# Agricultural-Robotics-Bonn/pagnerf

Measured on AMD Instinct MI355X. Metric: rays/sec (train step) on BUP20-shape scene, higher is better.
Workload: dtype bf16

## Files before the change

include/pagnerf_hip.h:

```cpp
#ifndef PAGNERF_HIP_H
#define PAGNERF_HIP_H

#include <stdint.h>

#ifdef __cplusplus
extern "C" {
#endif

#define PAG_ABI_VERSION 14

enum { PAG_F32 = 0, PAG_F16 = 1, PAG_BF16 = 2 };
enum { PAG_OK = 0, PAG_ERR_ARG = -1, PAG_ERR_LAUNCH = -2, PAG_ERR_UNSUPPORTED = -3 };
enum { PAG_ACT_NONE = 0, PAG_ACT_SIGMOID = 1, PAG_ACT_SOFTMAX = 2 };
enum { PAG_MLP_MFMA_BF16 = 0, PAG_MLP_FP32 = 1 };
enum { PAG_BG_BLACK = 0, PAG_BG_WHITE = 1 };
enum { PAG_LAYOUT_STRIDED = 0, PAG_LAYOUT_XCD8 = 1 };
enum { PAG_ENC_HALF_COORDS = 1 };
#define PAG_MAX_LEVELS 32
#define PAG_MAX_FEATS 64

int pag_abi_version(void);
const char *pag_last_error_string(void);


// ... 44 lines not shown
                            float *d_xyz, void *workspace, int64_t workspace_bytes, int flags, void *stream);
int pag_permuto_encode_bwd_xyz(const float *xyz, int64_t M, const void *tables, int table_dtype,
                               const void *grad_out, int grad_dtype, int64_t g_stride_m,
                               int64_t g_stride_c, int layout, int n_levels, int n_feat,
                               uint32_t capacity, const float *scale_factor_host,
                               const float *shift_host, const float *feat_scale_host, float *d_xyz,
                               void *workspace, int64_t workspace_bytes, int flags, void *stream);

int64_t pag_encode_bwd_workspace_bytes(int64_t M, int n_levels, int n_feat, int n_vertices,
                                       int64_t rows_per_level);


struct pag_head_composite_args;
typedef struct pag_mlp_fwd_args {
    const void *x1; int x1_dtype; int k1;
    int x1_layout; int x1_levels; int x1_feats;
    const float *x2; int k2p; const int32_t *x2_index;
    int in_dim; int n_layers; int out_dim;
    const float *W[3]; const float *b[3];
    int out_act;
    void *out; int out_dtype;
    void *hidden_save[2];
    int mode;
    float *softmax_stats;
    float *x1_col0_relu;
    const struct pag_mlp_fwd_args *pair;
    const struct pag_head_composite_args *composite;
    const struct pag_mlp_fwd_args *x1_producer;
} pag_mlp_fwd_args;
typedef struct pag_head_composite_args {
    const int64_t *pack_start; const int32_t *ray_of_pack; int64_t P;
    const float *weights;
    const float *alpha;
    float *out;
    int64_t n_samples;
} pag_head_composite_args;
int pag_mlp_fwd(const pag_mlp_fwd_args *args, int64_t M, void *stream);
int pag_mlp_fwd_pair_supported(const pag_mlp_fwd_args *args, const pag_mlp_fwd_args *pair);
int pag_mlp_fwd_composite_supported(const pag_mlp_fwd_args *args, int64_t M);
int pag_mlp_fwd_producer_supported(const pag_mlp_fwd_args *args, const pag_mlp_fwd_args *producer, int64_t M);

typedef struct pag_mlp_bwd_args {
    const void *grad_out; const void *out; int out_dtype; int out_act;
    int k1; int in_dim; int n_layers; int out_dim;
    int x1_layout; int x1_levels; int x1_feats;
    const float *W[3];
    const void *hidden_save[2];
    void *dz[3];
    void *dx1; int dx1_dtype;
    int mode;
    const float *g_ray; const float *g_scale; const int32_t *g_index;
    const float *softmax_stats; const float *b_last;
    int dx1_accumulate;
    const float *dx1_col0_add;
    const float *dx1_col0_gate;
    const float *g_ray_scale;
    const void *x1; int x1_dtype; const float *x2; int k2p; const int32_t *x2_index;
    float *wgrad_workspace; int64_t wgrad_workspace_bytes;
    float *dW[3]; float *db[3];
    const float *b[3];
    const struct pag_mlp_bwd_args *pair;
    float *dz0_slots;
} pag_mlp_bwd_args;
int pag_mlp_bwd(const pag_mlp_bwd_args *args, int64_t M, void *stream);
int64_t pag_mlp_dz0_slots_bytes(int64_t M, int64_t R);
int pag_mlp_dz0_slots_sum(const int64_t *pack_start, int64_t R, const float *slots, float *out, void *stream);
int pag_mlp_bwd_fused_supported(const pag_mlp_bwd_args *args);
#define PAG_MLP_FUSED_WIDE_MAX_M ((int64_t)1 << 24)
int64_t pag_mlp_bwd_fused_workspace_bytes(const pag_mlp_bwd_args *args, int64_t M);
int pag_mlp_bwd_pair_supported(const pag_mlp_bwd_args *args, const pag_mlp_bwd_args *pair);

int pag_affine_xcd8_fwd(const void *x, int64_t M, int x_levels, int x_feats, const float *W, const float *b, int n_out, int in_dim,
                        float *out, void *stream);
int pag_affine_xcd8_bwd_dx(const float *grad_out, int64_t M, int x_levels, int x_feats, const float *W, int n_out, int in_dim, void *dx,
                           void *stream);

int pag_head_composite_fwd(const int64_t *pack_start, const int32_t *ray_of_pack, int64_t P,
                           const void *hidden, const float *W_last, const float *b_last, int out_dim,
                           const float *softmax_stats, const float *weights, const float *alpha,
                           float *out, int64_t n_samples, void *stream);

int pag_mlp_wgrad_blocks(int64_t M);
int pag_mlp_wgrad(const void *dz, int dz_cols, int n_out, const void *a1, int a1_dtype,
                  int a1_layout, int k1, const float *a2, int k2p, const int32_t *a2_index, int n_in,
                  float *slabs, int n_blocks, int64_t M, void *stream);

int pag_mlp_wgrad_finish(const float *slabs, int n_blocks, int n_out, int n_in, int a1_layout,
                         int a1_levels, int a1_feats, float *dW, float *db, void *stream);

typedef struct pag_wgrad_layer {
    const void *dz;
    int dz_cols, n_out;
    const void *a1;
    int a1_dtype, a1_layout, k1;
    const float *a2;
    int k2p;
    const int32_t *a2_index;
    int n_in;
    float *slabs;
    int n_blocks;
    int a1_levels, a1_feats;
    float *dW, *db;
} pag_wgrad_layer;
int pag_mlp_wgrad_batch(const pag_wgrad_layer *layers, int n_layers, int64_t M, void *stream);


int pag_raymarch_count(const float *origins, const float *dirs, int64_t N, int S,
                       const float *tvals, const float *jitter, float dist_min, float dist_max,
                       const uint32_t *occupancy_bits, int blas_level, int32_t *counts,
                       void *stream);
int pag_pack_offsets(const int32_t *counts, int64_t N, int64_t *pack_start, int64_t *total_host, void *stream);
int pag_pad_packed(const int64_t *pack_start, int64_t N, int64_t capacity, int samples_per_entry, float *samples, float *depths,
                   float *deltas, int32_t *ridx_sample, int32_t *ridx_entry, int64_t *ridx64, int32_t *pidx,
                   uint8_t *boundary, int64_t *pack_start_clamped, void *stream);

int pag_pack_offsets_pad(const int32_t *counts, int64_t N, int64_t *pack_start, int64_t *total_host, int64_t capacity,
                         int samples_per_entry, float *samples, float *depths, float *deltas, int32_t *ridx_sample,
                         int32_t *ridx_entry, int64_t *ridx64, int32_t *pidx, uint8_t *boundary, int64_t *pack_start_clamped,
                         const float *dirs_src, float *dirs_dst, void *stream);

int pag_copy_batch(int n, void *const *dst, const void *const *src, const int64_t *nbytes, void *stream);

int pag_view_embed(const float *dirs, int64_t R, int n_freq, int width, float *out, void *stream);

int pag_raymarch_pack(const float *origins, const float *dirs, int64_t N, int S,
                      const float *tvals, const float *jitter, float dist_min, float dist_max,
                      const uint32_t *occupancy_bits, int blas_level, const int64_t *offsets,
                      int32_t *ridx, int32_t *pidx, float *samples, float *depths, float *deltas,
                      uint8_t *boundary, int64_t *ridx64, void *stream);

int pag_raymarch_voxel_count(const float *origins, const float *dirs, int64_t N, int samples_per_voxel,
                             float dist_min, float dist_max, const uint32_t *occupancy_bits,
                             const uint32_t *occupancy_coarse, int blas_level, float max_travel,
                             int32_t *counts, void *stream);
int pag_raymarch_voxel_pack(const float *origins, const float *dirs, int64_t N, int samples_per_voxel,
                            float dist_min, float dist_max, const uint32_t *occupancy_bits,
                            const uint32_t *occupancy_coarse, int blas_level, float max_travel,
                            const int64_t *offsets, int32_t *ridx, int32_t *pidx, float *samples,
                            float *depths, float *deltas, uint8_t *boundary, int32_t *ridx_sample,
                            int64_t *ridx64, void *stream);

int64_t pag_raymarch_voxel_nugget_capacity(int blas_level);
int pag_raymarch_voxel_count_nuggets(const float *origins, const float *dirs, int64_t N, int samples_per_voxel,
                                     float dist_min, float dist_max, const uint32_t *occupancy_bits,
                                     const uint32_t *occupancy_coarse, int blas_level, float max_travel,
                                     int32_t *counts, float *nugget_t, int32_t *nugget_cell, void *stream);
int pag_raymarch_voxel_pack_nuggets(const float *origins, const float *dirs, int64_t N, int samples_per_voxel,
                                    const int64_t *offsets, const float *nugget_t, const int32_t *nugget_cell, int blas_level,
                                    int32_t *ridx, int32_t *pidx, float *samples, float *depths, float *deltas,
                                    uint8_t *boundary, int32_t *ridx_sample, int64_t *ridx64, void *stream);

int64_t pag_occupancy_coarse_bytes(int blas_level);
int pag_occupancy_coarse(const uint32_t *occupancy_bits, int blas_level, uint32_t *coarse, void *stream);

int pag_occupancy_update(const float *density, int64_t density_stride, float *occupancy,
                         uint32_t *occupancy_bits, int64_t num_cells, float decay,
                         float min_density, void *stream);


int pag_composite_fwd(const int64_t *pack_start, const int32_t *ray_of_pack, int64_t P,
                      const float *sigma, const float *deltas, const float *depths,
                      const float *rgb, int bg_color, float *weights, float *out_alpha,
                      float *out_rgb, float *out_depth, uint8_t *out_hit, int64_t n_samples, void *stream);

int pag_composite_bwd(const int64_t *pack_start, const int32_t *ray_of_pack, int64_t P,
                      const float *sigma, const float *deltas, const float *depths,
                      const float *rgb, int bg_color, const float *weights,
                      const float *out_alpha, const float *g_rgb, const float *g_depth,
                      const float *g_alpha, float *d_sigma, float *d_rgb, int64_t n_samples, void *stream);

int pag_ray_sample_grad(const int64_t *pack_start, const int32_t *ray_of_pack, int64_t P, const float *grad_samples, const float *depths,
                        float *out, void *stream);

int pag_composite_feats_fwd(const int64_t *pack_start, const int32_t *ray_of_pack, int64_t P,
                            const float *weights, const float *alpha, const void *feats,
                            int feat_dtype, int C, float *out, void *stream);
int pag_composite_feats_bwd(const int64_t *pack_start, const int32_t *ray_of_pack, int64_t P,
                            const float *weights, const float *alpha, const float *g_out, int C,
                            void *d_feats, int feat_dtype, void *stream);


int pag_label_sums(const void *values, int value_dtype, int64_t P, int64_t row_stride, int col0, int C,
                   const int64_t *labels_gt, const uint8_t *row_mask, const int64_t *label_list, int K,
                   float *sums, int32_t *counts, void *stream);

int pag_assign_cost(const float *prob, int B, int64_t P, int64_t image_stride, int64_t row_stride, int n_cols, int col0,
                    const int64_t *labels_gt, int max_rows, float *sums_ws, int32_t *counts_ws, int32_t *info, int64_t *labels,
                    float *cost, const float *points, float id_slope, float id_x_limit, int id_margin, float *psums_ws,
                    int32_t *pcounts_ws, int32_t *id_lo_hi, void *stream);
int pag_assign_solve(const float *cost, int B, int max_rows, int n_ids, const int32_t *info, const int32_t *id_lo_hi, int64_t *targets, int32_t *status,
                     void *stream);
int pag_assign_nll_fwd(const float *prob, int B, int64_t P, int64_t image_stride, int64_t row_stride, int n_cols,
                       const int64_t *labels_gt, const uint8_t *stuff_mask, const int64_t *labels, const int64_t *targets,
                       const int32_t *info, int max_rows, int64_t default_label, int64_t *virt, float *loss, uint8_t *valid,
                       int32_t *wrong, void *stream);
int pag_assign_nll_bwd(const float *prob, int B, int64_t P, int64_t image_stride, int64_t row_stride, int n_cols,
                       const int64_t *virt, const uint8_t *valid, const int32_t *wrong, const float *grad, float *d_prob,
                       void *stream);

int64_t pag_segment_reg_workspace_bytes(int B, int64_t P);
int pag_segment_reg_fwd(const float *prob, int B, int64_t P, int64_t image_stride, int64_t row_stride, int n_cols, float eps,
                        const int64_t *labels, void *workspace, int64_t workspace_bytes, float *out, void *stream);
int pag_segment_reg_bwd(const float *prob, int B, int64_t P, int64_t image_stride, int64_t row_stride, int n_cols, float eps,
                        const void *workspace, int64_t workspace_bytes, const float *grad, float *d_prob, void *stream);


int64_t pag_supcon_workspace_bytes(int B, int64_t P, int D);
int pag_supcon_fwd(const void *features, int dtype, int B, int64_t P, int D, int64_t image_stride, int64_t row_stride, const int64_t *labels,
                   const uint8_t *anchor_mask, float temperature, float base_temperature, float pos_weight, float neg_weight, void *workspace,
                   int64_t workspace_bytes, float *loss, void *stream);
int pag_supcon_bwd(int dtype, int B, int64_t P, int D, float temperature, float base_temperature, float pos_weight, float neg_weight, void *workspace,
                   int64_t workspace_bytes, const float *grad_loss, void *d_features, void *stream);


int64_t pag_meanshift_workspace_bytes(int B, int64_t P, int D);

int pag_meanshift_fit(const void *features, int dtype, int B, int64_t P, int D, int64_t image_stride, int64_t row_stride, const int64_t *labels,
                      double quantile, int max_iter, int stages, void *workspace, int64_t workspace_bytes, float *means, double *bandwidth,
                      float *centers, int32_t *info, void *stream);

int pag_meanshift_predict(const void *x, int dtype, int64_t N, int D, int64_t row_stride, const float *centers, int C, int64_t *labels_out,
                          void *stream);

enum { PAG_I32 = 3, PAG_I64 = 4 };

int64_t pag_panoptic_pq_workspace_bytes(int B, int64_t H, int64_t W, int n_cat);

int pag_panoptic_pq_update(const void *preds, int preds_dtype, const int64_t *preds_strides, const void *target, int target_dtype,
                           const int64_t *target_strides, int B, int64_t H, int64_t W, const int64_t *cat_ids, const int32_t *cat_cont, int n_cat,
                           int n_things, int allow_unknown, void *workspace, int64_t workspace_bytes, double *iou_sum, int32_t *true_positives,
                           int32_t *false_positives, int32_t *false_negatives, int32_t *state_flags, void *stream);

int64_t pag_panoptic_clean_workspace_bytes(int64_t H, int64_t W);

int pag_panoptic_clean(const void *ids, int dtype, int64_t H, int64_t W, int64_t stride_y, int64_t stride_x, int num_openings, int outlier_rejection,
                       int64_t min_area, double std_threshold, void *workspace, int64_t workspace_bytes, void *out, void *stream);

int pag_confusion_matrix(const void *preds, int preds_dtype, const int64_t *preds_strides, const void *target, int target_dtype,
                         const int64_t *target_strides, const int64_t *shape, int C, int64_t *confmat, void *stream);


int64_t pag_map_workspace_bytes(int64_t n);

int pag_map_points(const float *params, int64_t C, const int32_t *cam, int64_t n_cam, int64_t rays_per_camera, const float *origins_c,
                   const float *dirs_c, int64_t ray0, int64_t n, const float *depth, const float *alpha, const uint8_t *hit,
                   const float *density, const float *rgb, const float *inst, int I, int64_t inst_stride, const int64_t *ids_in,
                   float min_density, float min_alpha, float depth_min, float depth_max, float *points, float *color, int64_t *ids_out,
                   int64_t cap, int64_t *count, void *workspace, int64_t workspace_bytes, void *stream);

int pag_map_select(const float *points_in, int64_t n, const float *value, float threshold, const float *inst, int I, int64_t inst_stride,
                   const int64_t *ids_in, float *points, int64_t *ids_out, int64_t cap, int64_t *count, void *workspace,
                   int64_t workspace_bytes, void *stream);


int64_t pag_render_loss_workspace_bytes(void);
int pag_render_loss_fwd(const float *rgb, const float *rgb_gt, int64_t N, float rgb_weight,
                        const float *prob_a, int C_a, const int64_t *target_a, const float *conf_a, float weight_a,
                        float inv_temp_a, int all_a,
                        const float *prob_b, int C_b, const int64_t *target_b, const float *conf_b, float weight_b,
                        float inv_temp_b, int all_b,
                        float eps, void *workspace, float *out, void *stream);

int pag_render_loss_bwd(const float *g, const float *fwd_out, const float *rgb, const float *rgb_gt, int64_t N,
                        float rgb_weight,
                        const float *prob_a, int C_a, const int64_t *target_a, const float *conf_a, float weight_a,
                        float inv_temp_a, int all_a,
                        const float *prob_b, int C_b, const int64_t *target_b, const float *conf_b, float weight_b,
                        float inv_temp_b, int all_b,
                        float eps, float *d_rgb, float *d_a, float *d_b, void *stream);

int pag_adam_step(int n_tensors, float *const *params, const float *const *grads, float *const *exp_avg, float *const *exp_avg_sq,
                  const int64_t *numel, double lr, double beta1, double beta2, double eps, double weight_decay, int64_t step,
                  void *stream);

int pag_pose_rays_fwd(const float *params, int64_t C, const int32_t *cam, int64_t rays_per_entry, const float *origins_c, const float *dirs_c,
                      int64_t N, float *origins_w, float *dirs_w, void *stream);
int64_t pag_pose_rays_bwd_workspace_bytes(int64_t C);
int pag_pose_rays_bwd(const float *params, int64_t C, const int32_t *cam, int64_t rays_per_entry, const float *origins_c, const float *dirs_c,
                      int64_t N, const float *g_origins, const float *g_dirs, float *d_params, void *workspace, int64_t workspace_bytes, void *stream);

int64_t pag_encode_bwd_rays_workspace_bytes(int64_t M, int64_t N);
int pag_hash_encode_bwd_rays(const float *xyz, int64_t M, const void *tables, int table_dtype, const void *grad_out, int grad_dtype,
                             int64_t g_stride_m, int64_t g_stride_c, int layout, int n_levels, int n_feat, int log2_T,
                             const float *resolutions_host, const float *feat_scale_host, const int32_t *ridx, const float *depths,
                             const int64_t *pack_start, int64_t N, float *out, void *workspace, int64_t workspace_bytes, int flags, void *stream);
int pag_permuto_encode_bwd_rays(const float *xyz, int64_t M, const void *tables, int table_dtype, const void *grad_out, int grad_dtype,
                                int64_t g_stride_m, int64_t g_stride_c, int layout, int n_levels, int n_feat, uint32_t capacity,
                                const float *scale_factor_host, const float *shift_host, const float *feat_scale_host, const int32_t *ridx,
                                const float *depths, const int64_t *pack_start, int64_t N, float *out, void *workspace, int64_t workspace_bytes,
                                int flags, void *stream);

int pag_pose_points(const float *params, int64_t C, const int32_t *cam, int64_t rays_per_entry, const float *origins_c, const float *dirs_c,
                    const float *depth, int64_t N, float *points, void *stream);

int pag_view_embed_bwd(const float *dirs, int64_t R, int n_freq, int width, const float *g_out, float *d_dirs, void *stream);

int pag_sparse_rows_mask(const float *grad, int L, int64_t T, int F, uint32_t *bits, void *stream);
int pag_sparse_rows_plan(const uint32_t *bits, int L, int64_t T, const int32_t *caps, int32_t *word_prefix, int64_t *counts, void *stream);
int pag_sparse_rows_pack(const float *grad, int L, int64_t T, int F, const uint32_t *bits, const int32_t *word_prefix, const int32_t *caps, const int64_t *offs,
                         float *buf, void *stream);
int pag_sparse_rows_unpack(const float *buf, int L, int64_t T, int F, const uint32_t *bits, const int32_t *word_prefix, const int32_t *caps, const int64_t *offs,
                           float *grad, void *stream);

#ifdef __cplusplus
}
#endif
#endif
```

pagnerf_amd/_lib.py:

```python
import ctypes
import os

import torch

from . import build as _build

F32, F16, BF16 = 0, 1, 2
I32, I64 = 3, 4
ACT_NONE, ACT_SIGMOID, ACT_SOFTMAX = 0, 1, 2
MLP_MFMA_BF16, MLP_FP32 = 0, 1
BG_BLACK, BG_WHITE = 0, 1
LAYOUT_STRIDED, LAYOUT_XCD8 = 0, 1
ENC_HALF_COORDS = 1
ABI_VERSION = 14
MLP_FUSED_WIDE_MAX_M = 1 << 24

_DT = {torch.float32: F32, torch.float16: F16, torch.bfloat16: BF16}

c_i64, c_i32, c_u32, c_f32, c_vp = ctypes.c_int64, ctypes.c_int, ctypes.c_uint32, ctypes.c_float, ctypes.c_void_p
c_fp = ctypes.POINTER(ctypes.c_float)


class HeadCompositeArgs(ctypes.Structure):
    _fields_ = [("pack_start", c_vp), ("ray_of_pack", c_vp), ("P", c_i64), ("weights", c_vp), ("alpha", c_vp), ("out", c_vp), ("n_samples", c_i64)]


class MlpFwdArgs(ctypes.Structure):
    pass


MlpFwdArgs._fields_ = [("x1", c_vp), ("x1_dtype", c_i32), ("k1", c_i32),
                ("x1_layout", c_i32), ("x1_levels", c_i32), ("x1_feats", c_i32),
                ("x2", c_vp), ("k2p", c_i32), ("x2_index", c_vp),
                ("in_dim", c_i32), ("n_layers", c_i32), ("out_dim", c_i32),
                ("W", c_vp * 3), ("b", c_vp * 3),
                ("out_act", c_i32),
                ("out", c_vp), ("out_dtype", c_i32),
                ("hidden_save", c_vp * 2),
                ("mode", c_i32),
                ("softmax_stats", c_vp), ("x1_col0_relu", c_vp), ("pair", ctypes.POINTER(MlpFwdArgs)),
                ("composite", ctypes.POINTER(HeadCompositeArgs)), ("x1_producer", ctypes.POINTER(MlpFwdArgs))]


class WgradLayer(ctypes.Structure):
    _fields_ = [("dz", c_vp), ("dz_cols", c_i32), ("n_out", c_i32),
                ("a1", c_vp), ("a1_dtype", c_i32), ("a1_layout", c_i32), ("k1", c_i32),
                ("a2", c_vp), ("k2p", c_i32), ("a2_index", c_vp), ("n_in", c_i32),
                ("slabs", c_vp), ("n_blocks", c_i32), ("a1_levels", c_i32), ("a1_feats", c_i32),
                ("dW", c_vp), ("db", c_vp)]


class MlpBwdArgs(ctypes.Structure):
    pass


MlpBwdArgs._fields_ = [("grad_out", c_vp), ("out", c_vp), ("out_dtype", c_i32), ("out_act", c_i32),
                ("k1", c_i32), ("in_dim", c_i32), ("n_layers", c_i32), ("out_dim", c_i32),
                ("x1_layout", c_i32), ("x1_levels", c_i32), ("x1_feats", c_i32),
                ("W", c_vp * 3),
                ("hidden_save", c_vp * 2),
                ("dz", c_vp * 3),
                ("dx1", c_vp), ("dx1_dtype", c_i32),
                ("mode", c_i32),
                ("g_ray", c_vp), ("g_scale", c_vp), ("g_index", c_vp),
                ("softmax_stats", c_vp), ("b_last", c_vp), ("dx1_accumulate", c_i32), ("dx1_col0_add", c_vp),
                ("dx1_col0_gate", c_vp), ("g_ray_scale", c_vp),
                ("x1", c_vp), ("x1_dtype", c_i32), ("x2", c_vp), ("k2p", c_i32), ("x2_index", c_vp),
                ("wgrad_workspace", c_vp), ("wgrad_workspace_bytes", c_i64),
                ("dW", c_vp * 3), ("db", c_vp * 3), ("b", c_vp * 3),
                ("pair", ctypes.POINTER(MlpBwdArgs)), ("dz0_slots", c_vp)]


_SIGS = {
    "pag_abi_version": (c_i32, []),
    "pag_last_error_string": (ctypes.c_char_p, []),
    "pag_hash_encode_fwd": (c_i32, [c_vp, c_i64, c_vp, c_i32, c_i32, c_i32, c_i32, c_fp, c_fp, c_vp, c_i32, c_i64, c_i64, c_i32, c_i32, c_vp]),
    "pag_hash_encode_bwd": (c_i32, [c_vp, c_i64, c_vp, c_i32, c_i64, c_i64, c_i32, c_i32, c_i32, c_i32, c_fp, c_fp, c_vp, c_vp, c_i64, c_i32, c_vp]),
    "pag_hash_encode_bwd_set": (c_i32, [c_vp, c_i64, c_vp, c_i32, c_i64, c_i64, c_i32, c_i32, c_i32, c_i32, c_fp, c_fp, c_vp, c_vp, c_i64, c_i32, c_vp]),
    "pag_permuto_encode_fwd": (c_i32, [c_vp, c_i64, c_vp, c_i32, c_i32, c_i32, c_u32, c_fp, c_fp, c_fp, c_vp, c_i32, c_i64, c_i64, c_i32, c_i32, c_vp]),
    "pag_permuto_encode_bwd": (c_i32, [c_vp, c_i64, c_vp, c_i32, c_i64, c_i64, c_i32, c_i32, c_i32, c_u32, c_fp, c_fp, c_fp, c_vp, c_vp, c_i64, c_i32, c_vp]),
    "pag_permuto_encode_bwd_set": (c_i32, [c_vp, c_i64, c_vp, c_i32, c_i64, c_i64, c_i32, c_i32, c_i32, c_u32, c_fp, c_fp, c_fp, c_vp, c_vp, c_i64, c_i32, c_vp]),
    "pag_hash_encode_bwd_xyz": (c_i32, [c_vp, c_i64, c_vp, c_i32, c_vp, c_i32, c_i64, c_i64, c_i32, c_i32, c_i32, c_i32, c_fp, c_fp, c_vp, c_vp, c_i64, c_i32, c_vp]),
    "pag_permuto_encode_bwd_xyz": (c_i32, [c_vp, c_i64, c_vp, c_i32, c_vp, c_i32, c_i64, c_i64, c_i32, c_i32, c_i32, c_u32, c_fp, c_fp, c_fp, c_vp, c_vp, c_i64, c_i32, c_vp]),
    "pag_hash_encode_fwd_add": (c_i32, [c_vp, c_i64, c_vp, c_i32, c_i32, c_i32, c_i32, c_fp, c_fp, c_vp, c_vp, c_i32, c_vp]),
    "pag_permuto_encode_fwd_add": (c_i32, [c_vp, c_i64, c_vp, c_i32, c_i32, c_i32, c_u32, c_fp, c_fp, c_fp, c_vp, c_vp, c_i32, c_vp]),
    "pag_encode_bwd_workspace_bytes": (c_i64, [c_i64, c_i32, c_i32, c_i32, c_i64]),
    "pag_mlp_fwd": (c_i32, [ctypes.POINTER(MlpFwdArgs), c_i64, c_vp]),
    "pag_mlp_fwd_pair_supported": (c_i32, [ctypes.POINTER(MlpFwdArgs), ctypes.POINTER(MlpFwdArgs)]),
    "pag_mlp_fwd_composite_supported": (c_i32, [ctypes.POINTER(MlpFwdArgs), c_i64]),
    "pag_mlp_fwd_producer_supported": (c_i32, [ctypes.POINTER(MlpFwdArgs), ctypes.POINTER(MlpFwdArgs), c_i64]),
    "pag_mlp_bwd": (c_i32, [ctypes.POINTER(MlpBwdArgs), c_i64, c_vp]),
    "pag_mlp_bwd_fused_supported": (c_i32, [ctypes.POINTER(MlpBwdArgs)]),
    "pag_mlp_bwd_fused_workspace_bytes": (c_i64, [ctypes.POINTER(MlpBwdArgs), c_i64]),
    "pag_mlp_bwd_pair_supported": (c_i32, [ctypes.POINTER(MlpBwdArgs), ctypes.POINTER(MlpBwdArgs)]),
    "pag_head_composite_fwd": (c_i32, [c_vp, c_vp, c_i64, c_vp, c_vp, c_vp, c_i32, c_vp, c_vp, c_vp, c_vp, c_i64, c_vp]),
    "pag_mlp_wgrad_blocks": (c_i32, [c_i64]),
    "pag_mlp_wgrad_batch": (c_i32, [ctypes.POINTER(WgradLayer), c_i32, c_i64, c_vp]),
    "pag_mlp_wgrad_finish": (c_i32, [c_vp, c_i32, c_i32, c_i32, c_i32, c_i32, c_i32, c_vp, c_vp, c_vp]),
    "pag_mlp_wgrad": (c_i32, [c_vp, c_i32, c_i32, c_vp, c_i32, c_i32, c_i32, c_vp, c_i32, c_vp, c_i32, c_vp, c_i32, c_i64, c_vp]),
    "pag_raymarch_count": (c_i32, [c_vp, c_vp, c_i64, c_i32, c_vp, c_vp, c_f32, c_f32, c_vp, c_i32, c_vp, c_vp]),
    "pag_pack_offsets": (c_i32, [c_vp, c_i64, c_vp, c_vp, c_vp]),
    "pag_pad_packed": (c_i32, [c_vp, c_i64, c_i64, c_i32, c_vp, c_vp, c_vp, c_vp, c_vp, c_vp, c_vp, c_vp, c_vp, c_vp]),
    "pag_view_embed": (c_i32, [c_vp, c_i64, c_i32, c_i32, c_vp, c_vp]),
    "pag_raymarch_pack": (c_i32, [c_vp, c_vp, c_i64, c_i32, c_vp, c_vp, c_f32, c_f32, c_vp, c_i32, c_vp, c_vp, c_vp, c_vp, c_vp, c_vp, c_vp, c_vp, c_vp]),
    "pag_raymarch_voxel_count": (c_i32, [c_vp, c_vp, c_i64, c_i32, c_f32, c_f32, c_vp, c_vp, c_i32, c_f32, c_vp, c_vp]),
    "pag_raymarch_voxel_pack": (c_i32, [c_vp, c_vp, c_i64, c_i32, c_f32, c_f32, c_vp, c_vp, c_i32, c_f32, c_vp, c_vp, c_vp, c_vp, c_vp, c_vp, c_vp,
                                        c_vp, c_vp, c_vp]),
    "pag_raymarch_voxel_nugget_capacity": (c_i64, [c_i32]),
    "pag_raymarch_voxel_count_nuggets": (c_i32, [c_vp, c_vp, c_i64, c_i32, c_f32, c_f32, c_vp, c_vp, c_i32, c_f32, c_vp, c_vp, c_vp, c_vp]),
    "pag_raymarch_voxel_pack_nuggets": (c_i32, [c_vp, c_vp, c_i64, c_i32, c_vp, c_vp, c_vp, c_i32, c_vp, c_vp, c_vp, c_vp, c_vp, c_vp, c_vp, c_vp, c_vp]),
    "pag_ray_sample_grad": (c_i32, [c_vp, c_vp, c_i64, c_vp, c_vp, c_vp, c_vp]),
    "pag_affine_xcd8_fwd": (c_i32, [c_vp, c_i64, c_i32, c_i32, c_vp, c_vp, c_i32, c_i32, c_vp, c_vp]),
    "pag_affine_xcd8_bwd_dx": (c_i32, [c_vp, c_i64, c_i32, c_i32, c_vp, c_i32, c_i32, c_vp, c_vp]),
    "pag_occupancy_coarse_bytes": (c_i64, [c_i32]),
    "pag_occupancy_coarse": (c_i32, [c_vp, c_i32, c_vp, c_vp]),
    "pag_occupancy_update": (c_i32, [c_vp, c_i64, c_vp, c_vp, c_i64, c_f32, c_f32, c_vp]),
    "pag_label_sums": (c_i32, [c_vp, c_i32, c_i64, c_i64, c_i32, c_i32, c_vp, c_vp, c_vp, c_i32, c_vp, c_vp, c_vp]),
    "pag_assign_cost": (c_i32, [c_vp, c_i32, c_i64, c_i64, c_i64, c_i32, c_i32, c_vp, c_i32, c_vp, c_vp, c_vp, c_vp, c_vp, c_vp, ctypes.c_float, ctypes.c_float, c_i32,
                                c_vp, c_vp, c_vp, c_vp]),
    "pag_sparse_rows_mask": (c_i32, [c_vp, c_i32, c_i64, c_i32, c_vp, c_vp]),
    "pag_sparse_rows_plan": (c_i32, [c_vp, c_i32, c_i64, c_vp, c_vp, c_vp, c_vp]),
    "pag_sparse_rows_pack": (c_i32, [c_vp, c_i32, c_i64, c_i32, c_vp, c_vp, c_vp, c_vp, c_vp, c_vp]),
    "pag_sparse_rows_unpack": (c_i32, [c_vp, c_i32, c_i64, c_i32, c_vp, c_vp, c_vp, c_vp, c_vp, c_vp]),
    "pag_assign_solve": (c_i32, [c_vp, c_i32, c_i32, c_i32, c_vp, c_vp, c_vp, c_vp, c_vp]),
    "pag_assign_nll_fwd": (c_i32, [c_vp, c_i32, c_i64, c_i64, c_i64, c_i32, c_vp, c_vp, c_vp, c_vp, c_vp, c_i32, c_i64, c_vp, c_vp, c_vp, c_vp, c_vp]),
    "pag_assign_nll_bwd": (c_i32, [c_vp, c_i32, c_i64, c_i64, c_i64, c_i32, c_vp, c_vp, c_vp, c_vp, c_vp, c_vp]),
    "pag_render_loss_workspace_bytes": (c_i64, []),
    "pag_render_loss_fwd": (c_i32, [c_vp, c_vp, c_i64, c_f32, c_vp, c_i32, c_vp, c_vp, c_f32, c_f32, c_i32, c_vp, c_i32, c_vp, c_vp, c_f32, c_f32, c_i32, c_f32, c_vp, c_vp, c_vp]),
    "pag_render_loss_bwd": (c_i32, [c_vp, c_vp, c_vp, c_vp, c_i64, c_f32, c_vp, c_i32, c_vp, c_vp, c_f32, c_f32, c_i32, c_vp, c_i32, c_vp, c_vp, c_f32, c_f32, c_i32, c_f32, c_vp, c_vp, c_vp, c_vp]),
    "pag_composite_fwd": (c_i32, [c_vp, c_vp, c_i64, c_vp, c_vp, c_vp, c_vp, c_i32, c_vp, c_vp, c_vp, c_vp, c_vp, c_i64, c_vp]),
    "pag_composite_bwd": (c_i32, [c_vp, c_vp, c_i64, c_vp, c_vp, c_vp, c_vp, c_i32, c_vp, c_vp, c_vp, c_vp, c_vp, c_vp, c_vp, c_i64, c_vp]),
    "pag_composite_feats_fwd": (c_i32, [c_vp, c_vp, c_i64, c_vp, c_vp, c_vp, c_i32, c_i32, c_vp, c_vp]),
    "pag_composite_feats_bwd": (c_i32, [c_vp, c_vp, c_i64, c_vp, c_vp, c_vp, c_i32, c_vp, c_i32, c_vp]),
    "pag_pack_offsets_pad": (c_i32, [c_vp, c_i64, c_vp, c_vp, c_i64, c_i32, c_vp, c_vp, c_vp, c_vp, c_vp, c_vp, c_vp, c_vp, c_vp, c_vp, c_vp, c_vp]),
    "pag_copy_batch": (c_i32, [c_i32, c_vp, c_vp, c_vp, c_vp]),
    "pag_adam_step": (c_i32, [c_i32, c_vp, c_vp, c_vp, c_vp, c_vp, ctypes.c_double, ctypes.c_double, ctypes.c_double, ctypes.c_double,
                              ctypes.c_double, c_i64, c_vp]),
    "pag_pose_rays_fwd": (c_i32, [c_vp, c_i64, c_vp, c_i64, c_vp, c_vp, c_i64, c_vp, c_vp, c_vp]),
    "pag_pose_rays_bwd_workspace_bytes": (c_i64, [c_i64]),
    "pag_pose_rays_bwd": (c_i32, [c_vp, c_i64, c_vp, c_i64, c_vp, c_vp, c_i64, c_vp, c_vp, c_vp, c_vp, c_i64, c_vp]),
    "pag_view_embed_bwd": (c_i32, [c_vp, c_i64, c_i32, c_i32, c_vp, c_vp, c_vp]),
    "pag_pose_points": (c_i32, [c_vp, c_i64, c_vp, c_i64, c_vp, c_vp, c_vp, c_i64, c_vp, c_vp]),
    "pag_segment_reg_workspace_bytes": (c_i64, [c_i32, c_i64]),
    "pag_segment_reg_fwd": (c_i32, [c_vp, c_i32, c_i64, c_i64, c_i64, c_i32, ctypes.c_float, c_vp, c_vp, c_i64, c_vp, c_vp]),
    "pag_segment_reg_bwd": (c_i32, [c_vp, c_i32, c_i64, c_i64, c_i64, c_i32, ctypes.c_float, c_vp, c_i64, c_vp, c_vp, c_vp]),
    "pag_supcon_workspace_bytes": (c_i64, [c_i32, c_i64, c_i32]),
    "pag_supcon_fwd": (c_i32, [c_vp, c_i32, c_i32, c_i64, c_i32, c_i64, c_i64, c_vp, c_vp, c_f32, c_f32, c_f32, c_f32, c_vp, c_i64, c_vp, c_vp]),
    "pag_supcon_bwd": (c_i32, [c_i32, c_i32, c_i64, c_i32, c_f32, c_f32, c_f32, c_f32, c_vp, c_i64, c_vp, c_vp, c_vp]),
    "pag_meanshift_workspace_bytes": (c_i64, [c_i32, c_i64, c_i32]),
    "pag_meanshift_fit": (c_i32, [c_vp, c_i32, c_i32, c_i64, c_i32, c_i64, c_i64, c_vp, ctypes.c_double, c_i32, c_i32, c_vp, c_i64, c_vp, c_vp, c_vp, c_vp,
                                  c_vp]),
    "pag_meanshift_predict": (c_i32, [c_vp, c_i32, c_i64, c_i32, c_i64, c_vp, c_i32, c_vp, c_vp]),
    "pag_panoptic_pq_workspace_bytes": (c_i64, [c_i32, c_i64, c_i64, c_i32]),
    "pag_panoptic_pq_update": (c_i32, [c_vp, c_i32, c_vp, c_vp, c_i32, c_vp, c_i32, c_i64, c_i64, c_vp, c_vp, c_i32, c_i32, c_i32, c_vp, c_i64, c_vp, c_vp,
                                       c_vp, c_vp, c_vp, c_vp]),
    "pag_panoptic_clean_workspace_bytes": (c_i64, [c_i64, c_i64]),
    "pag_panoptic_clean": (c_i32, [c_vp, c_i32, c_i64, c_i64, c_i64, c_i64, c_i32, c_i32, c_i64, ctypes.c_double, c_vp, c_i64, c_vp, c_vp]),
    "pag_confusion_matrix": (c_i32, [c_vp, c_i32, c_vp, c_vp, c_i32, c_vp, c_vp, c_i32, c_vp, c_vp]),
    "pag_map_workspace_bytes": (c_i64, [c_i64]),
    "pag_map_points": (c_i32, [c_vp, c_i64, c_vp, c_i64, c_i64, c_vp, c_vp, c_i64, c_i64, c_vp, c_vp, c_vp, c_vp, c_vp, c_vp, c_i32, c_i64, c_vp,
                               c_f32, c_f32, c_f32, c_f32, c_vp, c_vp, c_vp, c_i64, c_vp, c_vp, c_i64, c_vp]),
    "pag_map_select": (c_i32, [c_vp, c_i64, c_vp, c_f32, c_vp, c_i32, c_i64, c_vp, c_vp, c_vp, c_i64, c_vp, c_vp, c_i64, c_vp]),
    "pag_mlp_dz0_slots_bytes": (c_i64, [c_i64, c_i64]),
    "pag_mlp_dz0_slots_sum": (c_i32, [c_vp, c_i64, c_vp, c_vp, c_vp]),
    "pag_encode_bwd_rays_workspace_bytes": (c_i64, [c_i64, c_i64]),
    "pag_hash_encode_bwd_rays": (c_i32, [c_vp, c_i64, c_vp, c_i32, c_vp, c_i32, c_i64, c_i64, c_i32, c_i32, c_i32, c_i32, c_fp, c_fp, c_vp, c_vp, c_vp, c_i64,
                                         c_vp, c_vp, c_i64, c_i32, c_vp]),
    "pag_permuto_encode_bwd_rays": (c_i32, [c_vp, c_i64, c_vp, c_i32, c_vp, c_i32, c_i64, c_i64, c_i32, c_i32, c_i32, c_u32, c_fp, c_fp, c_fp, c_vp, c_vp, c_vp,
                                            c_i64, c_vp, c_vp, c_i64, c_i32, c_vp]),
}

EXPORTS = tuple(_SIGS)
_lib = None


def load():
    global _lib
    if _lib is None:
        path = _build.LIB
        if not os.path.exists(path):
            raise RuntimeError("libpagnerf_hip.so not found at %s - run `python -m pagnerf_amd.build` "
                               "(there is no CPU fallback for the HIP path)" % path)
        lib = ctypes.CDLL(path)
        for name, (res, args) in _SIGS.items():
            fn = getattr(lib, name)
            fn.restype = res
            fn.argtypes = args
        if lib.pag_abi_version() != ABI_VERSION:
            raise RuntimeError("libpagnerf_hip.so ABI version mismatch")
        _lib = lib
    return _lib


def check(rc, name):
    if rc != 0:
        msg = load().pag_last_error_string().decode("utf-8", "replace")
        raise RuntimeError("%s failed (%d): %s" % (name, rc, msg))


def dtype_code(t):
    return _DT[t.dtype]


def ptr(t):
    if t is None:
        return None
    if not t.is_cuda:
        raise RuntimeError("pagnerf_amd: expected a GPU tensor (the HIP path has no CPU fallback), got %s" % t.device)
    if not t.is_contiguous():
        raise RuntimeError("pagnerf_amd: tensor must be contiguous")
    return t.data_ptr()


_RAW_STREAM = getattr(torch._C, "_cuda_getCurrentRawStream", None)


def stream():
    if _RAW_STREAM is not None:
        return _RAW_STREAM(torch.cuda.current_device())
    return torch.cuda.current_stream().cuda_stream


def host_floats(values):
    if values is None:
        return None
    if isinstance(values, torch.Tensor):
        values = values.detach().cpu().float().reshape(-1).tolist()
    else:
        import numpy as np
        values = np.asarray(values, dtype=np.float32).reshape(-1).tolist()
    return (ctypes.c_float * len(values))(*values)
```

pagnerf_amd/build.py:

```python
import concurrent.futures
import hashlib
import os
import subprocess
import sys

HERE = os.path.dirname(os.path.abspath(__file__))
CSRC = os.path.join(HERE, "csrc")
LIBDIR = os.path.join(HERE, "lib")
LIB = os.path.join(LIBDIR, "libpagnerf_hip.so")
ARCH = "gfx950"

COMMON = ["--offload-arch=" + ARCH, "-O3", "-fPIC", "-std=c++17", "-munsafe-fp-atomics", "-Wno-unused-value"]
MLP = ["-mllvm", "-amdgpu-mfma-vgpr-form=1"]
SOURCES = {
    "mlp.hip": MLP,
    "encode.hip": ["-ffp-contract=off"],
    "mlp_wgrad.hip": MLP,
    "render.hip": ["-ffp-contract=off"],
    "mlp_affine.hip": MLP,
    "api.cpp": ["-x", "hip"],
    "assign.hip": ["-ffp-contract=off"],
    "loss.hip": ["-ffp-contract=off"],
    "optim.hip": ["-ffp-contract=off"],
    "pose.hip": ["-ffp-contract=off"],
    "regularizer.hip": ["-ffp-contract=off"],
    "supcon.hip": ["-ffp-contract=off"],
    "cluster.hip": ["-ffp-contract=off"],
    "panoptic.hip": ["-ffp-contract=off"],
    "map.hip": ["-ffp-contract=off"],
    "sparse.hip": [],
}


def _jobs():
    n = min(16, os.cpu_count() or 4)
    try:
        n = min(n, int(os.environ.get("MAX_JOBS", "")))
    except ValueError:
        pass
    return max(1, n)


def _hipcc():
    for c in (os.environ.get("HIPCC"), "/opt/rocm/bin/hipcc", "hipcc"):
        if c and (os.path.isabs(c) and os.path.exists(c) or not os.path.isabs(c)):
            return c
    raise RuntimeError("hipcc not found")


_COMPILER_ID = None


def _compiler_id():
    global _COMPILER_ID
    if _COMPILER_ID is None:
        try:
            out = subprocess.run([_hipcc(), "--version"], capture_output=True, text=True, timeout=120).stdout
        except Exception as e:
            out = "unavailable: %r" % (e,)
        _COMPILER_ID = "\n".join(l.strip() for l in out.splitlines() if l.startswith(("HIP version", "AMD clang version"))) or out.strip()
    return _COMPILER_ID


def _digest():
    h = hashlib.sha256()
    h.update(repr((COMMON, sorted(SOURCES.items()))).encode())
    h.update(_compiler_id().encode())
    for root in (CSRC, os.path.join(os.path.dirname(HERE), "include")):
        for f in sorted(os.listdir(root)):
            if not os.path.isfile(os.path.join(root, f)):
                continue
            with open(os.path.join(root, f), "rb") as fh:
                h.update(f.encode())
                h.update(fh.read())
    return h.hexdigest()


def _compile(src, flags, obj):
    cmd = [_hipcc()] + COMMON + flags + ["-c", os.path.join(CSRC, src), "-o", obj]
    r = subprocess.run(cmd, capture_output=True, text=True)
    if r.returncode != 0:
        raise RuntimeError("hipcc failed for %s:\n%s\n%s" % (src, " ".join(cmd), r.stderr[-4000:]))
    return src


def build(force=False, verbose=True):
    os.makedirs(os.path.join(LIBDIR, "obj"), exist_ok=True)
    stamp = os.path.join(LIBDIR, "build.sha256")
    dig = _digest()
    if not force and os.path.exists(LIB) and os.path.exists(stamp) and open(stamp).read().strip() == dig:
        if verbose:
            print("[pagnerf_amd.build] up to date:", LIB, file=sys.stderr)
        return LIB
    objs = {s: os.path.join(LIBDIR, "obj", os.path.splitext(s)[0] + ".o") for s in SOURCES}
    with concurrent.futures.ThreadPoolExecutor(max_workers=_jobs()) as ex:
        futs = [ex.submit(_compile, s, f, objs[s]) for s, f in SOURCES.items()]
        for f in concurrent.futures.as_completed(futs):
            if verbose:
                print("[pagnerf_amd.build] compiled", f.result(), file=sys.stderr)
    cmd = [_hipcc(), "--offload-arch=" + ARCH, "-shared", "-fPIC", "-o", LIB] + list(objs.values())
    r = subprocess.run(cmd, capture_output=True, text=True)
    if r.returncode != 0:
        raise RuntimeError("link failed:\n%s" % r.stderr[-4000:])
    with open(stamp, "w") as fh:
        fh.write(dig)
    if verbose:
        print("[pagnerf_amd.build] linked", LIB, file=sys.stderr)
    return LIB


if __name__ == "__main__":
    build(force="--force" in sys.argv)
```

pagnerf_amd/graphs.py:

```python
import collections
import os
import weakref

import torch
import torch.nn as nn

from . import ops
from .core import RenderBuffer

GRANULE = 8192
HEADROOM = 1.02
HISTORY = 8
CAP_STEPS = 32
SHRINK_WINDOW = 64
MAX_BUCKETS = 2


def _round_capacity(want, k):
    gran = GRANULE * k
    step = max(gran, (1 << (max(int(want), 1).bit_length() - 1)) // CAP_STEPS // gran * gran)
    return (int(want) + step - 1) // step * step


class _PostMarch(nn.Module):

    def __init__(self, nef, tracer, buf, capacity, channels, lod_idx, bg_color, stage):
        super().__init__()
        self.nef = nef
        self._t = (tracer, buf)
        self.capacity, self.channels, self.lod_idx, self.bg_color, self.stage = capacity, frozenset(channels), lod_idx, bg_color, stage
        self.names = None

    def forward(self, samples, depths, deltas, ray_dirs, origins=None):
        tracer, buf = self._t
        cap, k, N = self.capacity, buf.k, buf.N
        ne = cap // k
        smp = samples.reshape(ne, k, 3)
        dep = depths.reshape(ne, k)
        if origins is not None:
            smp = ops.ray_samples(origins, ray_dirs, smp, dep, buf.pack_start_c, ops._ray_iota(N, samples.device), ridx=buf.ridx_sample[:cap])
        out = tracer.shade(self.nef, set(self.channels), set(), ray_dirs, N, buf.ridx_entry[:ne], buf.ridx_sample[:cap], buf.pidx[:ne], smp, dep,
                           deltas, buf.pack_start_c, ops._ray_iota(N, samples.device), self.lod_idx, self.bg_color, self.stage)
        if self.names is None:
            self.names = sorted(out)
        return tuple(out[n] for n in self.names)


def _fresh(statics):
    outs = [torch.empty_like(o, memory_format=torch.contiguous_format) for o in statics]
    if outs:
        ops.copy_batch(outs, list(statics))
    return outs


class _GraphedFn(torch.autograd.Function):

    @staticmethod
    def forward(ctx, runner, gi, *params):
        ctx.runner, ctx.gi = runner, gi
        ctx.set_materialize_grads(False)
        grp = runner.groups[gi]
        ctx.generation = runner.generation
        idx = grp.out_idx + (runner.nondiff_idx if gi == 0 else [])
        outs = _fresh([runner.outs[i] for i in idx])
        ctx.mark_non_differentiable(*outs[len(grp.out_idx):])
        return tuple(outs)

    @staticmethod
    @torch.autograd.function.once_differentiable
    def backward(ctx, *grads):
        r = ctx.runner
        grp = r.groups[ctx.gi]
        if ctx.generation != r.generation:
            raise RuntimeError("pagnerf_amd.graphs: the forward graph of this configuration was replayed again before this backward ran - the "
                               "activations it saved are gone.  Call backward() on a trace before tracing the same configuration again "
                               "(or construct the tracer with use_graphs=False / 'static').")
        r.detach_param_grads(grp)
        dst, src, zero = [], [], []
        for i, (static, g) in enumerate(zip(grp.gouts, grads)):
            if g is None:
                if i not in grp.zeroed:
                    zero.append(static)
                    grp.zeroed.add(i)
            else:
                dst.append(static)
                src.append(g if (g.dtype == static.dtype and g.shape == static.shape) else g.to(static.dtype).reshape(static.shape))
                grp.zeroed.discard(i)
        if zero:
            torch._foreach_zero_(zero)
        if dst:
            ops.copy_batch(dst, src)
        grp.bwd.replay()
        n_p = len(grp.params)
        return (None, None) + tuple(g.detach() for g in grp.gins[:n_p]) + tuple(_fresh(grp.gins[n_p:]))


class _Group:
    __slots__ = ("out_idx", "gouts", "bwd", "gins", "params", "zeroed", "arg_sel")


class _Graphed:

    def __init__(self, mod, args, split=(), grad_args=()):
        self.mod = mod
        named = [(n, p) for n, p in mod.named_parameters() if p.requires_grad]
        params = [p for _, p in named]
        cur = torch.cuda.current_stream()
        side = torch.cuda.Stream()
        side.wait_stream(cur)
        with torch.cuda.stream(side):
            self.alias = {n: p.detach().requires_grad_(True) for n, p in named}
            args = tuple(a.detach().requires_grad_(True) if i in grad_args else a for i, a in enumerate(args))
        self.args = args
        self.grad_args = tuple(grad_args)
        leaves = list(self.alias.values()) + [args[i] for i in grad_args]

        def run():
            return torch.func.functional_call(mod, self.alias, args)

        def groups_of(outs):
            diff = [i for i, o in enumerate(outs) if o.requires_grad]
            late = [i for i in diff if mod.names[i] in split]
            rest = [i for i in diff if mod.names[i] not in split]
            return [g for g in (late, rest) if g] or [[]]
        with torch.cuda.stream(side):
            for _ in range(2):
                outs = run()
                gs = groups_of(outs)
                for j, idx in enumerate(gs):
                    if idx:
                        torch.autograd.grad([outs[i] for i in idx], leaves, [torch.zeros_like(outs[i]) for i in idx], allow_unused=True,
                                            retain_graph=j + 1 < len(gs))
                del outs
        cur.wait_stream(side)
        torch.cuda.synchronize()
        pool = torch.cuda.graph_pool_handle()
        self.fwd = torch.cuda.CUDAGraph()
        with torch.cuda.graph(self.fwd, pool=pool):
            self.outs = run()
        self.nondiff_idx = [i for i, o in enumerate(self.outs) if not o.requires_grad]
        self.groups = []
        gs = groups_of(self.outs)
        for j, idx in enumerate(gs):
            grp = _Group()
            grp.out_idx = idx
            grp.gouts = [torch.zeros_like(self.outs[i]) for i in idx]
            grp.zeroed = set()
            grp.bwd = torch.cuda.CUDAGraph()
            if idx:
                with torch.cuda.graph(grp.bwd, pool=pool if len(gs) == 1 else torch.cuda.graph_pool_handle()):
                    gins = torch.autograd.grad([self.outs[i] for i in idx], leaves, grp.gouts, allow_unused=True, retain_graph=j + 1 < len(gs))
            else:
                gins = [None] * len(leaves)
            used = [i for i, g in enumerate(gins) if g is not None]
            grp.params = [params[i] for i in used if i < len(params)]
            grp.arg_sel = [i - len(params) for i in used if i >= len(params)]
            grp.gins = [gins[i] for i in used]
            self.groups.append(grp)
        self.generation = 0
        self.unaliased = 0
        torch.cuda.synchronize()

    def detach_param_grads(self, grp=None):
        for g_ in ([grp] if grp is not None else self.groups):
            for p, g in zip(g_.params, g_.gins):
                pg = p.grad
                if pg is not None and pg.untyped_storage().data_ptr() == g.untyped_storage().data_ptr():
                    p.grad = pg.clone()
                    self.unaliased += 1

    def __call__(self, live_args=()):
        assert len(live_args) == len(self.grad_args)
        self.detach_param_grads()
        self.fwd.replay()
        self.generation += 1
        res = [None] * len(self.outs)
        for gi in reversed(range(len(self.groups))):
            grp = self.groups[gi]
            outs = _GraphedFn.apply(self, gi, *grp.params, *[live_args[j] for j in grp.arg_sel])
            for i, o in zip(grp.out_idx + (self.nondiff_idx if gi == 0 else []), outs):
                res[i] = o
        return tuple(res)


class _State:
    def __init__(self):
        self.counts = collections.deque(maxlen=HISTORY)
        self.long = collections.deque(maxlen=SHRINK_WINDOW)
        self.cap = None
        self.buf = None
        self.dirs = None
        self.orig0 = None
        self.buckets = collections.OrderedDict()

    def see(self, count):
        self.counts.append(int(count))
        self.long.append(int(count))

    def capacity(self, buf):
        want = _round_capacity(int(max(self.counts) * HEADROOM) + 1, buf.k)
        if self.cap is None or want > self.cap:
            self.cap = want
            self.long.clear()
        elif len(self.long) == self.long.maxlen:
            small = _round_capacity(int(max(self.long) * HEADROOM) + 1, buf.k)
            if small < self.cap:
                self.cap = small
                self.long.clear()
        self.cap = min(buf.cap, self.cap)
        return self.cap

    def bucket(self, key, make=None):
        b = self.buckets.get(key)
        if b is not None:
            self.buckets.move_to_end(key)
            return b
        if make is None:
            return None
        while len(self.buckets) >= MAX_BUCKETS:
            self.buckets.popitem(last=False)
        b = self.buckets[key] = make()
        return b


class GraphRunner:

    MAX_STATES = 4

    def __init__(self):
        self.states = collections.OrderedDict()
        self.replays = self.captures = self.overflows = 0

    def _state(self, key):
        st = self.states.get(key)
        if st is None:
            while len(self.states) >= self.MAX_STATES:
                self.states.popitem(last=False)
            st = self.states[key] = _State()
        else:
            self.states.move_to_end(key)
        return st

    @staticmethod
    def _split(tracer):
        force = getattr(tracer, "graph_split", None)
        if force is None:
            force = os.environ.get("PAG_GRAPH_SPLIT", "") not in ("", "0")
        multi = torch.distributed.is_available() and torch.distributed.is_initialized() and torch.distributed.get_world_size() > 1
        return tuple(sorted(tracer.panoptic_channels)) if (force or multi) else ()

    @staticmethod
    def eligible(tracer, nef, channels, extra_channels, rays, stage):
        if not torch.is_grad_enabled() or stage != "train" or extra_channels or tracer.ray_sparcity_reg > 0.0:
            return False
        if not rays.origins.is_cuda:
            return False
        if not getattr(nef, "accepts_ray_index", False) or not getattr(nef.grid, "accepts_max_travel", False):
            return False
        return True

    PARAM_RESCAN = 64
    MAX_SLOT_CACHES = 4

    @staticmethod
    def _structure(nef, mods):
        out = [(len(m._parameters), *m._modules.values()) for m in mods]
        out.append((len(nef._parameters), *nef._modules.values()))
        return out

    def _param_sig(self, nef):
        caches = self.__dict__.setdefault("_slot_caches", collections.OrderedDict())
        for k in [k for k, c in caches.items() if c[0]() is None]:
            del caches[k]
        cache = caches.get(id(nef))
        if cache is not None and (cache[0]() is not nef or cache[2] <= 0 or self._structure(nef, cache[3]) != cache[4]):
            cache = None
        if cache is None:
            mods = [m for m in nef.modules() if m is not nef]
            slots = [(m, n) for m in mods for n, p in m._parameters.items() if p is not None]
            own = [n for n, p in nef._parameters.items() if p is not None]
            cache = caches[id(nef)] = [weakref.ref(nef), slots, self.PARAM_RESCAN, mods, self._structure(nef, mods), own]
            while len(caches) > self.MAX_SLOT_CACHES:
                caches.popitem(last=False)
        caches.move_to_end(id(nef))
        cache[2] -= 1
        try:
            sig = [(m._parameters[n].data_ptr(), m._parameters[n].requires_grad) for m, n in cache[1]]
            sig += [(nef._parameters[n].data_ptr(), nef._parameters[n].requires_grad) for n in cache[5]]
            return tuple(sig)
        except (KeyError, AttributeError):
            caches.pop(id(nef), None)
            return self._param_sig(nef)

    def _key(self, tracer, nef, channels, rays, lod_idx, raymarch_type, num_steps, bg_color, stage):
        lw = nef.lod_weights
        grids = [nef.grid] + ([nef.delta_grid] if hasattr(nef, "delta_grid") else [])
        return (id(nef), raymarch_type, int(rays.origins.shape[0]), int(num_steps), frozenset(channels), lod_idx, bg_color, stage, nef.precision,
                nef.training, id(lw), lw._version, tuple((id(g.tables), g.tables.dtype, g.rounds_coords(), g.blas_level) for g in grids),
                float(rays.dist_min), float(rays.dist_max), float(tracer.ray_max_travel), str(rays.origins.device),
                self._param_sig(nef), self._split(tracer), bool(rays.origins.requires_grad or rays.dirs.requires_grad))

    def observe(self, key, count):
        self._state(key).see(count)

    def run(self, tracer, nef, channels, rays, lod_idx, raymarch_type, num_steps, bg_color, stage, jitter):
        key = self._key(tracer, nef, channels, rays, lod_idx, raymarch_type, num_steps, bg_color, stage)
        st = self._state(key)
        if not st.counts:
            return None, key, jitter
        g = nef.grid
        dev = rays.origins.device
        N = rays.origins.shape[0]
        if st.buf is None:
            if raymarch_type == "ray":
                st.buf = ops.MarchBuffers("ray", N, num_steps, 1, dev)
            else:
                st.buf = ops.MarchBuffers("voxel", N, int(ops.L.load().pag_raymarch_voxel_nugget_capacity(g.blas_level)), int(num_steps), dev)
            st.dirs = torch.empty(N, 3, device=dev)
        pose = bool(rays.origins.requires_grad or rays.dirs.requires_grad)
        if pose and st.orig0 is None:
            st.orig0 = torch.zeros(N, 3, device=dev)
        buf = st.buf
        cap = st.capacity(buf)
        bits = None if g._all_occupied else g.blas_bits
        if bits is not None and bits.device != dev:
            g.blas_bits = bits = bits.to(dev)
        coarse = g._coarse_bits(bits) if (bits is not None and raymarch_type == "voxel") else None
        mailbox, jitter = ops.march_into(buf, rays.origins, rays.dirs, rays.dist_min, rays.dist_max, num_steps, jitter=jitter,
                                         occupancy_bits=bits, blas_level=g.blas_level,
                                         max_travel=tracer.ray_max_travel if raymarch_type == "voxel" else None, occupancy_coarse_bits=coarse,
                                         pad_capacity=cap, dirs_out=st.dirs)
        args = (buf.samples[:cap], buf.depths[:cap], buf.deltas[:cap], st.dirs) + ((st.orig0,) if pose else ())
        live = (rays.dirs, rays.origins) if pose else ()
        if tracer.use_graphs == "static":
            mod = st.bucket(("static", cap), lambda: _PostMarch(nef, tracer, buf, cap, channels, lod_idx, bg_color, stage))
            ops.SAMPLES_HINT, ops.TAIL_ZERO = max(st.counts), True
            try:
                outs = mod(*args[:3], *live) if pose else mod(*args)
            finally:
                ops.SAMPLES_HINT, ops.TAIL_ZERO = None, False
            self.replays += 1
            M = self._count(mailbox, buf)
            st.see(M)
            if M > cap:
                self.overflows += 1
                return None, key, jitter
            return RenderBuffer(**dict(zip(mod.names, outs))), key, jitter
        graphed = st.bucket(cap)
        if graphed is None:
            M = self._count(mailbox, buf)
            mailbox = None
            st.see(M)
            if M > cap:
                return None, key, jitter
            import gc
            for attr in ("_density_feats", "_feat_cache", "_prefetched"):
                if hasattr(nef, attr):
                    setattr(nef, attr, None)
            for grid in [nef.grid] + ([nef.delta_grid] if hasattr(nef, "delta_grid") else []):
                grid._pack_cache = None
            while len(st.buckets) >= MAX_BUCKETS:
                st.buckets.popitem(last=False)
            gc.collect()
            torch.cuda.synchronize()
            mod = _PostMarch(nef, tracer, buf, cap, channels, lod_idx, bg_color, stage)
            mod.train(nef.training)
            ops.SAMPLES_HINT = M
            ops.TAIL_ZERO = True
            try:
                graphed = st.bucket(cap, lambda: _Graphed(mod, args, split=self._split(tracer), grad_args=(3, 4) if pose else ()))
            finally:
                ops.SAMPLES_HINT, ops.TAIL_ZERO = None, False
            self.captures += 1
        outs = graphed(live)
        self.replays += 1
        if mailbox is not None:
            M = self._count(mailbox, buf)
            st.see(M)
            if M > cap:
                self.overflows += 1
                return None, key, jitter
        return RenderBuffer(**dict(zip(graphed.mod.names, outs))), key, jitter

    @staticmethod
    def _count(mailbox, buf):
        M = ops._poll_count(mailbox) if mailbox is not None else -1
        if mailbox is not None and M >= 0:
            ops._release_mailbox(mailbox)
        if M < 0:
            M = int(buf.counts.sum().item())
        return M
```

pagnerf_amd/nef.py:

```python
import copy
import inspect
import os

import numpy as np
import torch
import torch.nn as nn
import torch.nn.functional as F

from . import _lib as L
from . import ops
from .grids import HashGridHIP, PermutoGridHIP

_GRIDS = {"HashGridTorch": HashGridHIP, "HashGridTinyCudaNN": HashGridHIP, "HashGrid": HashGridHIP,
          "HashGridHIP": HashGridHIP, "PermutoGrid": PermutoGridHIP, "PermutoGridHIP": PermutoGridHIP}


class BasicDecoder(nn.Module):

    def __init__(self, input_dim, output_dim, num_layers=1, hidden_dim=64, bias=True):
        super().__init__()
        if hidden_dim != 64 or num_layers not in (1, 2):
            raise NotImplementedError("fused decoder supports hidden_dim=64 and 1-2 hidden layers (best.yaml); got %d x %d"
                                      % (num_layers, hidden_dim))
        self.input_dim, self.output_dim = input_dim, output_dim
        self.layers = nn.ModuleList([nn.Linear(input_dim if i == 0 else hidden_dim, hidden_dim, bias=bias)
                                     for i in range(num_layers)])
        self.lout = nn.Linear(hidden_dim, output_dim, bias=bias)

    def weights(self):
        lins = list(self.layers) + [self.lout]
        return [l.weight for l in lins], [l.bias for l in lins]

    def forward(self, x1, x2=None, x2_index=None, out_act=L.ACT_NONE, mode=L.MLP_MFMA_BF16, out_dtype=torch.float32,
                x1_grouped=None, x2_packs=None):
        W, b = self.weights()
        return ops.fused_mlp(x1, W, b, x2=x2, x2_index=x2_index, in_dim=self.input_dim, out_act=out_act, mode=mode,
                             out_dtype=out_dtype, x1_grouped=x1_grouped, x2_packs=x2_packs)


_PARAM_NAMES = {}


def _param_names(fn):
    key = getattr(fn, "__func__", fn)
    names = _PARAM_NAMES.get(key)
    if names is None:
        names = _PARAM_NAMES[key] = frozenset(inspect.signature(fn).parameters)
    return names


def positional_embed(x, num_freq):
    bands = 2.0 ** torch.linspace(0.0, num_freq - 1, num_freq, device=x.device)
    w = (x[:, None, :] * bands[None, :, None]).reshape(x.shape[0], num_freq * x.shape[-1])
    return torch.cat([x, torch.sin(w), torch.cos(w)], dim=-1)


class PanopticDeltaNeF(nn.Module):
    accepts_ray_index = True

    def __init__(self, grid_type="PermutoGrid", interpolation_type="linear", multiscale_type="cat", feature_dim=2,
                 num_lods=24, base_lod=2, hidden_dim=64, num_layers=1, activation_type="relu", layer_type="none",
                 embedder_type="positional", view_multires=4, pos_multires=4, position_input=False,
                 num_classes=-1, num_instances=-1,
                 sem_activation_type=None, sem_num_layers=None, sem_hidden_dim=None, sem_normalize=False,
                 sem_softmax=False, sem_sigmoid=False, sem_detach=True,
                 inst_num_layers=None, inst_hidden_dim=None, inst_normalize=False, inst_softmax=False,
                 inst_sigmoid=False, inst_detach=True, panoptic_features_type=None,
                 delta_num_layers=1, delta_hidden_dim=64, inst_soft_temperature=0.0,
                 raymarch_type="ray", precision="bf16", **kwargs):
        super().__init__()
        if activation_type != "relu" or (sem_activation_type or "relu") != "relu":
            raise NotImplementedError("fused decoders implement ReLU hidden activations (best.yaml)")
        if position_input:
            raise NotImplementedError
        if panoptic_features_type not in (None, "delta", "separate", "appearance", "pos_encoding", "position"):
            raise ValueError('Panoptic feature type "%s" not implemented for PanopticDeltaNeF' % panoptic_features_type)
        if multiscale_type not in ("cat", "sum"):
            raise NotImplementedError("'%s' not supported by this neural field. supported options ['cat', 'sum']" % multiscale_type)
        self.grid_type, self.multiscale_type = grid_type, multiscale_type
        self.feature_dim, self.num_lods, self.base_lod = feature_dim, num_lods, base_lod
        self.hidden_dim, self.num_layers = hidden_dim, num_layers
        self.view_multires, self.embedder_type = view_multires, embedder_type
        self.num_classes, self.num_instances = num_classes, num_instances
        self.sem_normalize, self.sem_softmax, self.sem_sigmoid = sem_normalize, sem_softmax, sem_sigmoid
        self.inst_normalize, self.inst_softmax, self.inst_sigmoid = inst_normalize, inst_softmax, inst_sigmoid
        self.panoptic_features_type = panoptic_features_type
        self.inst_soft_temperature = inst_soft_temperature
        self.raymarch_type = raymarch_type
        self.kwargs = kwargs
        self.set_precision(precision)
        gkw = dict(kwargs)
        gkw.pop("num_lods", None)
        if grid_type == "HashGridTinyCudaNN":
            gkw.setdefault("half_coords", True)
        self.grid = _GRIDS[grid_type](feature_dim, base_lod=base_lod, num_lods=num_lods,
                                      interpolation_type=interpolation_type, multiscale_type="cat", **gkw)
        self.lod_weights = torch.ones(num_lods * feature_dim)
        if panoptic_features_type in ("delta", "separate", None):
            self.delta_grid = copy.deepcopy(self.grid)
            if isinstance(self.delta_grid, PermutoGridHIP) and panoptic_features_type in ("delta", "separate") \
                    and "delta_capacity_log_2" in kwargs:
                self.delta_grid.set_capacity(kwargs["delta_capacity_log_2"])
        self.view_embed_dim = 3 + 6 * view_multires if embedder_type == "positional" else 3
        self.pos_multires, self.pos_embed_dim = pos_multires, 3 + 6 * pos_multires
        eff = feature_dim * num_lods if multiscale_type == "cat" else feature_dim
        pan_dim = {"position": 3, "pos_encoding": self.pos_embed_dim}.get(panoptic_features_type, eff)
        self.decoder_density = BasicDecoder(eff, 16, num_layers, hidden_dim)
        with torch.no_grad():
            self.decoder_density.lout.bias[0] = 1.0
        self.decoder_color = BasicDecoder(16 + self.view_embed_dim, 3, num_layers + 1, hidden_dim)
        self.decoder_semantics = BasicDecoder(pan_dim, num_classes, sem_num_layers or num_layers, sem_hidden_dim or hidden_dim)
        assert num_instances > 2
        self.decoder_inst = BasicDecoder(pan_dim, num_instances, inst_num_layers or num_layers, inst_hidden_dim or hidden_dim)
        self._fns = [(self.rgb_semantics, {"density", "rgb", "semantics", "inst_embedding"})]

    def set_precision(self, precision):
        assert precision in ("bf16", "fp32")
        self.precision = precision
        self.mlp_mode = L.MLP_MFMA_BF16 if precision == "bf16" else L.MLP_FP32
        self.feat_dtype = torch.bfloat16 if precision == "bf16" else torch.float32

    @property
    def device(self):
        return self.decoder_density.lout.weight.device

    def get_nef_type(self):
        return "delta_panoptic_nef"

    def get_supported_channels(self):
        s = set()
        for _, c in self._fns:
            s |= c
        return s

    def forward(self, channels=None, **kwargs):
        kwargs["compute_channels"] = channels
        req = {channels} if isinstance(channels, str) else set(channels)
        unsupported = req - self.get_supported_channels()
        if unsupported:
            raise Exception("Channels %s are not supported in %s" % (unsupported, type(self).__name__))
        out = {}
        for fn, chans in self._fns:
            if not (chans & req):
                continue
            params = _param_names(fn)
            res = fn(**{k: v for k, v in kwargs.items() if k in params})
            for c in chans & req:
                out[c] = res[c]
        if isinstance(channels, str):
            return out[channels]
        if isinstance(channels, list):
            return [out[c] for c in channels]
        return out

    def _view_embedding(self, ray_d, ridx, ray_dirs):
        if ray_dirs is not None and ridx is not None:
            src, index = ray_dirs, ridx
        else:
            src, index = ray_d, torch.arange(ray_d.shape[0], device=ray_d.device, dtype=torch.int32)
        if self.embedder_type == "positional" and src.is_cuda:
            width = 3 + 6 * self.view_multires
            width += (-width) % 8
            if src.requires_grad and torch.is_grad_enabled():
                return ops.view_embed_grad(src, self.view_multires, width), index
            return ops.view_embed(src, self.view_multires, width), index
        pe = positional_embed(-src.float(), self.view_multires) if self.embedder_type == "positional" else -src.float()
        return F.pad(pe, (0, (-pe.shape[1]) % 8)).contiguous(), index

    def _grouped(self):
        if self.precision == "bf16" and self.multiscale_type == "cat" and ops.xcd8_supported(self.num_lods, self.feature_dim):
            return (self.num_lods, self.feature_dim)
        return None

    def _pan_grouped(self):
        return None if self.panoptic_features_type in ("pos_encoding", "position") else self._grouped()

    @staticmethod
    def _pad8(x, dtype):
        return F.pad(x, (0, (-x.shape[1]) % 8)).to(dtype).contiguous()

    def _lod_weights_or_none(self):
        lw = self.lod_weights
        key = (id(lw), lw._version)
        if getattr(self, "_lw_key", None) != key:
            self._lw_key, self._lw_ones = key, bool((lw == 1).all())
        return None if self._lw_ones else lw

    def _interp(self, grid, coords, addend=None):
        lw = self._lod_weights_or_none()
        feats = grid.interpolate_scaled(coords, lw, out_dtype=self.feat_dtype, layout="xcd8" if self._grouped() else None,
                                        addend=addend)
        if self.multiscale_type == "sum":
            feats = self._pad8(feats.float().reshape(-1, self.num_lods, self.feature_dim).sum(-2), self.feat_dtype)
        return feats

    def prefetch_features(self, coords):
        if self.multiscale_type != "cat" or self.grid is None:
            return
        self._prefetched = (coords, self._interp(self.grid, coords), torch.is_grad_enabled())

    def _panoptic_feats(self, feats_detached, coords):
        t = self.panoptic_features_type
        if t == "pos_encoding":
            return self._pad8(positional_embed(coords.reshape(-1, 3).float(), self.pos_multires), self.feat_dtype)
        if t == "position":
            return self._pad8(coords.reshape(-1, 3).float(), self.feat_dtype)
        if t == "appearance":
            return feats_detached
        if t == "separate":
            return self._interp(self.delta_grid, coords.detach())
        if self._grouped() is not None:
            return self._interp(self.delta_grid, coords.detach(), addend=feats_detached)
        return feats_detached + self._interp(self.delta_grid, coords.detach())

    def rgb_semantics(self, coords, ray_d=None, compute_channels=None, pidx=None, lod_idx=None, ridx=None, ray_dirs=None,
                      ray_packs=None):
        out = {}
        if not compute_channels:
            return out
        if isinstance(compute_channels, str):
            compute_channels = {compute_channels}
        batch, num_samples, _ = coords.shape
        mode = self.mlp_mode
        pre = getattr(self, "_prefetched", None)
        self._prefetched = None
        if pre is not None and pre[0] is coords and pre[2] == torch.is_grad_enabled():
            feats = pre[1]
        else:
            feats = self._interp(self.grid, coords)
        self._feat_cache = (coords, feats if self._heads_read_live_features() else feats.detach())
        grp = self._grouped()
        hold = ops.decoder_hold(feats) if (ops.CD_FUSED and "rgb" in compute_channels and feats.is_cuda) else None
        try:
            density_feats = self.decoder_density(feats, mode=mode, out_dtype=self.feat_dtype, x1_grouped=grp)
            self._density_feats = density_feats.detach()
            if "rgb" in compute_channels:
                if num_samples != 1 and ridx is None:
                    ray_d = ray_d[:, None].repeat(1, num_samples, 1).reshape(-1, 3)
                pe, index = self._view_embedding(ray_d, ridx, ray_dirs)
                W, b = self.decoder_color.weights()
                rgb, sigma = ops.colour_and_density(density_feats, W, b, pe, index, self.decoder_color.input_dim, out_act=L.ACT_SIGMOID,
                                                    mode=mode, x2_packs=ray_packs if ridx is not None else None, producer=hold)
                density = sigma.reshape(batch, num_samples, 1)
                out["rgb"] = rgb.reshape(batch, num_samples, 3)
            else:
                density = torch.relu(density_feats[:, 0:1].float()).reshape(batch, num_samples, 1)
        finally:
            ops.flush_hold(hold)
        if "density" in compute_channels:
            out["density"] = density
        if "semantics" in compute_channels or "inst_embedding" in compute_channels:
            (sem_in, sem_grp), (inst_in, inst_grp) = self._head_inputs(feats, coords, compute_channels)
            if "semantics" in compute_channels:
                plain = not (self.sem_sigmoid or self.sem_normalize)
                act = L.ACT_SOFTMAX if (self.sem_softmax and plain) else L.ACT_NONE
                s = self.decoder_semantics(sem_in, out_act=act, mode=mode, x1_grouped=sem_grp, out_dtype=self.feat_dtype)
                if not plain:
                    s = torch.sigmoid(s) if self.sem_sigmoid else s
                    s = F.normalize(s, dim=-1) if self.sem_normalize else s
                    s = F.softmax(s, dim=-1) if self.sem_softmax else s
                out["semantics"] = s
            if "inst_embedding" in compute_channels:
                out["inst_embedding"] = self._inst_head(inst_in, inst_grp, mode)
        return out

    def _inst_head(self, inst_in, inst_grp, mode):
        plain = not (self.inst_sigmoid or self.inst_normalize or self.inst_soft_temperature > 0.0)
        act = L.ACT_SOFTMAX if (self.inst_softmax and plain) else L.ACT_NONE
        e = self.decoder_inst(inst_in, out_act=act, mode=mode, x1_grouped=inst_grp, out_dtype=self.feat_dtype)
        if not plain:
            e = torch.sigmoid(e) if self.inst_sigmoid else e
            e = F.normalize(e, dim=-1) if self.inst_normalize else e
            e = e / self.inst_soft_temperature if self.inst_soft_temperature > 0.0 else e
            e = F.softmax(e, dim=-1) if self.inst_softmax else e
        return e

    def _heads_read_live_features(self):
        return False

    def _head_inputs(self, feats, coords, channels):
        pan = self._panoptic_feats(feats.detach(), coords)
        grp = self._pan_grouped()
        return (pan, grp), (pan, grp)

    WIDE_HEAD_PAD = os.environ.get("PAG_WIDE_HEAD_PAD", "1") != "0"

    def _wide_head_weights(self, dec, x):
        W, b = dec.weights()
        if not (self.WIDE_HEAD_PAD and len(W) == 2 and x.is_cuda and self.precision == "bf16" and W[0].shape[0] == 64 and 192 < W[1].shape[0] <= 224
                and b[0] is not None and b[1] is not None):
            return W, b
        pad = getattr(self, "_wide_pad", None)
        if pad is None or pad[0].device != W[0].device:
            pad = self._wide_pad = (torch.eye(64, device=W[0].device), torch.zeros(64, device=W[0].device))
        return [W[0], pad[0], W[1]], [b[0], pad[1], b[1]]

    def can_fuse_panoptic(self, channels):
        if self.precision != "bf16" or self._pan_grouped() is None:
            return False
        ok = True
        if "semantics" in channels:
            ok &= self.sem_softmax and not (self.sem_sigmoid or self.sem_normalize)
        if "inst_embedding" in channels:
            ok &= self.inst_softmax and not (self.inst_sigmoid or self.inst_normalize or self.inst_soft_temperature > 0.0)
        return bool(ok)

    def panoptic_composited(self, coords, channels, w, alpha, ridx, pack_start, ray_of_pack, N):
        cache = getattr(self, "_feat_cache", None)
        self._feat_cache = None
        if cache is not None and cache[0] is coords:
            feats = cache[1]
        elif self._heads_read_live_features():
            feats = self._interp(self.grid, coords)
        else:
            with torch.no_grad():
                feats = self._interp(self.grid, coords)
        (sem_in, sem_grp), (inst_in, inst_grp) = self._head_inputs(feats, coords, channels)
        out = {}
        if "semantics" in channels and "inst_embedding" in channels and sem_in is inst_in and sem_grp is not None:
            heads = ((*self._wide_head_weights(self.decoder_inst, sem_in), self.decoder_inst.input_dim),
                     (*self.decoder_semantics.weights(), self.decoder_semantics.input_dim))
            out["inst_embedding"], out["semantics"] = ops.head_composite_pair(sem_in, heads, w, alpha, ridx, pack_start, ray_of_pack, N,
                                                                              out_dtype=self.feat_dtype, x1_grouped=sem_grp)
            return out
        for ch, dec, x, grp in (("semantics", self.decoder_semantics, sem_in, sem_grp), ("inst_embedding", self.decoder_inst, inst_in, inst_grp)):
            if ch in channels:
                W, b = self._wide_head_weights(dec, x) if ch == "inst_embedding" else dec.weights()
                out[ch] = ops.head_composite(x, W, b, w, alpha, ridx, pack_start, ray_of_pack, N, in_dim=dec.input_dim,
                                             out_act=L.ACT_SOFTMAX, out_dtype=self.feat_dtype, x1_grouped=grp)
        return out

    @torch.no_grad()
    def prune(self, jitter=None):
        if self.grid is None:
            return
        density_decay = 0.6
        min_density = (0.01 * 512) / np.sqrt(3)
        dev = self.device
        g = self.grid
        points = g.dense_points.to(dev)
        res = 2.0 ** g.blas_level
        if jitter is None:
            jitter = torch.rand(points.shape[0], 3, device=dev)
        samples = (points.float() + jitter) / res * 2.0 - 1.0
        views = torch.zeros(points.shape[0], 3, device=dev)
        views[:, 2] = 1.0
        with g.fp32_coords():
            density = self.forward(coords=samples[:, None], ray_d=views, channels="density")
        g.occupancy = g.occupancy.to(dev).float().contiguous()
        bits = torch.empty(max(1, (g.num_cells + 31) // 32), dtype=torch.int32, device=dev)
        ops.occupancy_update(density.reshape(-1), g.occupancy, bits, density_decay, min_density)
        for grid in [self.grid] + ([self.delta_grid] if hasattr(self, "delta_grid") else []):
            grid.blas_init_bits(bits)


class PanopticNeF(PanopticDeltaNeF):

    def __init__(self, *args, sem_detach=True, inst_detach=True, inst_direct_pos=False, panoptic_features_type=None, **kwargs):
        if panoptic_features_type == "pos_encoding":
            raise AttributeError("'PanopticNeF' object has no attribute 'pos_embed_dim'")
        super().__init__(*args, sem_detach=sem_detach, inst_detach=inst_detach,
                         panoptic_features_type="position" if panoptic_features_type == "position" else "appearance", **kwargs)
        self.panoptic_features_type = panoptic_features_type
        self.sem_detach, self.inst_detach, self.inst_direct_pos = bool(sem_detach), bool(inst_detach), bool(inst_direct_pos)
        if self.inst_soft_temperature > 0.0:
            raise NotImplementedError("inst_soft_temperature is an option of PanopticDeltaNeF only")

    def get_nef_type(self):
        return "panoptic_nef"

    def _pan_grouped(self):
        return self._grouped()

    def _heads_read_live_features(self):
        return not (self.sem_detach and (self.inst_detach or self.inst_direct_pos))

    def _head_inputs(self, feats, coords, channels):
        grp = self._grouped()
        if "semantics" in channels and self.panoptic_features_type == "position":
            raise RuntimeError("mat1 and mat2 shapes cannot be multiplied: PanopticNeF feeds its semantic head the grid features "
                               "(panoptic_nef.py:338) but panoptic_features_type='position' sized it for 3 inputs (:99-101)")
        det = feats.detach()
        sem = det if self.sem_detach else feats
        if self.inst_direct_pos:
            inst, inst_grp = self._pad8(coords.reshape(-1, 3).float(), self.feat_dtype), None
        else:
            inst = sem if self.inst_detach == self.sem_detach else (det if self.inst_detach else feats)
            inst_grp = grp
        return (sem, grp), (inst, inst_grp)

    def _inst_head(self, inst_in, inst_grp, mode):
        if self.inst_softmax:
            return self.decoder_inst(inst_in, out_act=L.ACT_SOFTMAX, mode=mode, x1_grouped=inst_grp, out_dtype=self.feat_dtype)
        e = self.decoder_inst(inst_in, out_act=L.ACT_NONE, mode=mode, x1_grouped=inst_grp, out_dtype=self.feat_dtype)
        e = torch.sigmoid(e) if self.inst_sigmoid else e
        return F.normalize(e, dim=-1) if self.inst_normalize else e

    def rgb_semantics(self, coords, ray_d=None, compute_channels=None, pidx=None, lod_idx=None, ridx=None, ray_dirs=None,
                      ray_packs=None):
        out = super().rgb_semantics(coords, ray_d=ray_d, compute_channels=compute_channels, pidx=pidx, lod_idx=lod_idx, ridx=ridx,
                                    ray_dirs=ray_dirs, ray_packs=ray_packs)
        if self.inst_direct_pos and "inst_embedding" in out:
            out["inst_embedding"] = out["inst_embedding"].reshape(coords.shape[0], coords.shape[1], -1)
        return out

    def can_fuse_panoptic(self, channels):
        if self.precision != "bf16" or self._grouped() is None:
            return False
        ok = True
        if "semantics" in channels:
            ok &= self.sem_softmax and not (self.sem_sigmoid or self.sem_normalize) and self.panoptic_features_type != "position"
        if "inst_embedding" in channels:
            ok &= self.inst_softmax and not self.inst_direct_pos
        return bool(ok)
```

pagnerf_amd/ops.py:

```python
import ctypes
import os
import threading
import time

import torch

from . import _lib as L


_PROFILE = None


_PROFILE_ONLY = None


def profile_start(only=None):
    global _PROFILE, _PROFILE_ONLY
    _PROFILE = {}
    _PROFILE_ONLY = set(only) if only is not None else None


def profile_stop():
    global _PROFILE
    prof, _PROFILE = _PROFILE, None
# ... 877 lines not shown
        _call("pag_view_embed", L.ptr(d), d.shape[0], int(n_freq), int(width), L.ptr(out), L.stream())
        return out

    @staticmethod
    def backward(ctx, g):
        (d,) = ctx.saved_tensors
        n_freq, width = ctx.cfg
        g = g.contiguous().float()
        out = torch.empty_like(d)
        _call("pag_view_embed_bwd", L.ptr(d), d.shape[0], n_freq, width, L.ptr(g), L.ptr(out), L.stream())
        return out, None, None


def view_embed_grad(dirs, n_freq, width):
    _check_gpu(dirs)
    return _apply(_ViewEmbed, dirs, n_freq, width)


class _PoseRays(torch.autograd.Function):

    @staticmethod
    def forward(ctx, params, cam, rays_per_entry, origins_c, dirs_c):
        p = params.detach().contiguous().float()
        oc, dc = origins_c.detach().contiguous().float(), dirs_c.detach().contiguous().float()
        N = oc.shape[0]
        ow, dw = torch.empty(N, 3, device=p.device), torch.empty(N, 3, device=p.device)
        _call("pag_pose_rays_fwd", L.ptr(p), p.shape[0], L.ptr(cam), int(rays_per_entry), L.ptr(oc), L.ptr(dc), N, L.ptr(ow), L.ptr(dw), L.stream())
        ctx.save_for_backward(p, cam, oc, dc)
        ctx.rpe = int(rays_per_entry)
        ctx.set_materialize_grads(False)
        return ow, dw

    @staticmethod
    def backward(ctx, g_o, g_d):
        p, cam, oc, dc = ctx.saved_tensors
        if g_o is None and g_d is None:
            return None, None, None, None, None
        g_o = g_o.contiguous().float() if g_o is not None else None
        g_d = g_d.contiguous().float() if g_d is not None else None
        d_params = torch.empty_like(p)
        ws_bytes = L.load().pag_pose_rays_bwd_workspace_bytes(p.shape[0])
        ws = torch.empty(ws_bytes // 4, device=p.device)
        _call("pag_pose_rays_bwd", L.ptr(p), p.shape[0], L.ptr(cam), ctx.rpe, L.ptr(oc), L.ptr(dc), oc.shape[0], L.ptr(g_o), L.ptr(g_d), L.ptr(d_params),
              L.ptr(ws), ws_bytes, L.stream())
        return d_params, None, None, None, None


def pose_rays(params, cam, rays_per_entry, origins_c, dirs_c):
    _check_gpu(params, cam, origins_c, dirs_c)
    if origins_c.shape != dirs_c.shape or origins_c.dim() != 2 or origins_c.shape[1] != 3:
        raise RuntimeError("pose_rays: origins / dirs must both be [N,3], got %s and %s" % (tuple(origins_c.shape), tuple(dirs_c.shape)))
    n_entries = (origins_c.shape[0] + rays_per_entry - 1) // rays_per_entry
    if cam.dtype != torch.int32 or cam.numel() < n_entries or params.dim() != 2 or params.shape[1] != 9:
        raise RuntimeError("pose_rays: cam must be int32 with one entry per %d rays, params [C,9]" % rays_per_entry)
    return _PoseRays.apply(params, cam.contiguous(), int(rays_per_entry), origins_c, dirs_c)


def pose_points(params, cam, rays_per_entry, origins_c, dirs_c, depth):
    _check_gpu(params, cam, origins_c, dirs_c, depth)
    N = origins_c.shape[0]
    if origins_c.shape != dirs_c.shape or origins_c.dim() != 2 or origins_c.shape[1] != 3 or depth.numel() != N:
        raise RuntimeError("pose_points: origins / dirs [N,3] and depth [N], got %s, %s, %s" % (tuple(origins_c.shape), tuple(dirs_c.shape), tuple(depth.shape)))
    n_entries = (N + rays_per_entry - 1) // rays_per_entry
    if cam.dtype != torch.int32 or cam.numel() < n_entries or params.dim() != 2 or params.shape[1] != 9:
        raise RuntimeError("pose_points: cam must be int32 with one entry per %d rays, params [C,9]" % rays_per_entry)
    prm, oc, dc = params.detach().contiguous().float(), origins_c.detach().contiguous().float(), dirs_c.detach().contiguous().float()
    dep = depth.detach().reshape(-1).contiguous().float()
    out = torch.empty(N, 3, device=oc.device)
    _call("pag_pose_points", prm.data_ptr(), prm.shape[0], cam.contiguous().data_ptr(), int(rays_per_entry), oc.data_ptr(), dc.data_ptr(), dep.data_ptr(), N,
          out.data_ptr(), L.stream())
    return out


class _RaySamples(torch.autograd.Function):

    @staticmethod
    def forward(ctx, origins, dirs, samples, depths, pack_start, ray_of_pack):
        ctx.save_for_backward(depths, pack_start, ray_of_pack)
        ctx.N = origins.shape[0]
        return samples.view_as(samples)

    @staticmethod
    def backward(ctx, g):
        depths, pack_start, ray_of_pack = ctx.saved_tensors
        N = ctx.N
        g = g.reshape(-1, 3).float().contiguous()
        P = ray_of_pack.shape[0]
        seg = (torch.empty if (P and _one_pack_per_ray(ray_of_pack, N)) else torch.zeros)(N, 6, device=g.device)
        if P and g.shape[0]:
            _call("pag_ray_sample_grad", L.ptr(pack_start), L.ptr(ray_of_pack), P, L.ptr(g), L.ptr(depths.reshape(-1).float().contiguous()),
                  L.ptr(seg), L.stream())
        elif P:
            seg.zero_()
        return seg[:, :3], seg[:, 3:], None, None, None, None


def ray_samples(origins, dirs, samples, depths, pack_start, ray_of_pack, ridx=None):
    out = _RaySamples.apply(origins, dirs, samples, depths, pack_start, ray_of_pack)
    if ridx is not None and _one_pack_per_ray(ray_of_pack, origins.shape[0]) and ridx.dtype == torch.int32:
        out._pag_rays = (origins, dirs, depths, pack_start, ridx)
    return out


_TVALS = {}


def _tvals(S, dev):
    key = (S, str(dev))
    if key not in _TVALS:
        _TVALS[key] = torch.linspace(0, 1.0, S).to(dev)
    return _TVALS[key]


def occupancy_coarse(occupancy_bits, blas_level):
    nbytes = L.load().pag_occupancy_coarse_bytes(int(blas_level))
    if occupancy_bits is None or nbytes == 0:
        return None
    coarse = torch.empty(nbytes // 4, device=occupancy_bits.device, dtype=torch.int32)
    _call("pag_occupancy_coarse", L.ptr(occupancy_bits), int(blas_level), L.ptr(coarse), L.stream())
    return coarse


VOXEL_SCRATCH_MAX = 1 << 30


def raymarch_voxel(origins, dirs, dist_min, dist_max, samples_per_voxel, occupancy_bits=None, blas_level=7, max_travel=None,
                   occupancy_coarse_bits=None, want_packs=False):
    return raymarch_voxel_finish(raymarch_voxel_begin(origins, dirs, dist_min, dist_max, samples_per_voxel, occupancy_bits, blas_level, max_travel,
                                                      occupancy_coarse_bits, want_packs))


def raymarch_voxel_begin(origins, dirs, dist_min, dist_max, samples_per_voxel, occupancy_bits=None, blas_level=7, max_travel=None,
                         occupancy_coarse_bits=None, want_packs=False):
    _check_gpu(origins, dirs)
    dev = origins.device
    N, k = origins.shape[0], int(samples_per_voxel)
    origins = origins.detach().contiguous().float()
    dirs = dirs.detach().contiguous().float()
    counts = torch.empty(N, device=dev, dtype=torch.int32)
    occ = L.ptr(occupancy_bits) if occupancy_bits is not None else None
    coarse = L.ptr(occupancy_coarse_bits) if (occupancy_coarse_bits is not None and occupancy_bits is not None) else None
    travel = float("inf") if max_travel is None else float(max_travel)
    st = L.stream()
    cap = int(L.load().pag_raymarch_voxel_nugget_capacity(blas_level))
    nug_t = nug_cell = None
    if N and 2 * cap * N * 12 <= VOXEL_SCRATCH_MAX:
        nug_t = torch.empty(2, cap, N, 2, device=dev)
        nug_cell = torch.empty(2, cap, N, device=dev, dtype=torch.int32)
        _call("pag_raymarch_voxel_count_nuggets", L.ptr(origins), L.ptr(dirs), N, k, float(dist_min), float(dist_max), occ, coarse,
              blas_level, travel, L.ptr(counts), L.ptr(nug_t), L.ptr(nug_cell), st)
    elif N:
        _call("pag_raymarch_voxel_count", L.ptr(origins), L.ptr(dirs), N, k, float(dist_min), float(dist_max), occ, coarse, blas_level,
              travel, L.ptr(counts), st)
    pack_start = torch.empty(N + 1, device=dev, dtype=torch.int64)
    mailbox = _count_mailbox() if POLL_SAMPLE_COUNT else None
    if mailbox is not None:
        mailbox[1][0] = -1
    _call("pag_pack_offsets", L.ptr(counts), N, L.ptr(pack_start), mailbox[0].data_ptr() if mailbox is not None else None, st)
    return (origins, dirs, N, k, float(dist_min), float(dist_max), occupancy_bits, occupancy_coarse_bits, occ, coarse, blas_level, travel, counts, nug_t, nug_cell,
            pack_start, mailbox, want_packs)


def raymarch_voxel_finish(state):
    (origins, dirs, N, k, dist_min, dist_max, _occ_t, _coarse_t, occ, coarse, blas_level, travel, counts, nug_t, nug_cell, pack_start, mailbox, want_packs) = state
    dev = origins.device
    st = L.stream()
    total = _poll_count(mailbox) if mailbox is not None else -1
    if total < 0:
        total = int(pack_start[N].item())
        if mailbox is not None and int(mailbox[1][0]) < 0:
            _disable_polling()
    if mailbox is not None and int(mailbox[1][0]) >= 0:
        _release_mailbox(mailbox)
    Mn = total // k
    ridx = torch.empty(Mn, device=dev, dtype=torch.int32)
    pidx = torch.empty(Mn, device=dev, dtype=torch.int32)
    samples = torch.empty(Mn, k, 3, device=dev)
    depths = torch.empty(Mn, k, device=dev)
    deltas = torch.empty(Mn * k, device=dev)
    boundary = torch.empty(Mn * k, device=dev, dtype=torch.uint8)
    ridx_sample = torch.empty(Mn * k, device=dev, dtype=torch.int32) if want_packs else None
    ridx64 = torch.empty(Mn, device=dev, dtype=torch.int64) if want_packs else None
    if Mn and nug_t is not None:
        _call("pag_raymarch_voxel_pack_nuggets", L.ptr(origins), L.ptr(dirs), N, k, L.ptr(pack_start), L.ptr(nug_t), L.ptr(nug_cell), blas_level,
              L.ptr(ridx), L.ptr(pidx), L.ptr(samples), L.ptr(depths), L.ptr(deltas), L.ptr(boundary), L.ptr(ridx_sample), L.ptr(ridx64), st)
    elif Mn:
        _call("pag_raymarch_voxel_pack", L.ptr(origins), L.ptr(dirs), N, k, dist_min, dist_max, occ, coarse, blas_level,
              travel, L.ptr(pack_start), L.ptr(ridx), L.ptr(pidx), L.ptr(samples), L.ptr(depths), L.ptr(deltas), L.ptr(boundary),
              L.ptr(ridx_sample), L.ptr(ridx64), st)
    if want_packs:
        return (ridx, pidx, samples, depths, deltas, boundary.view(torch.bool), pack_start, _ray_iota(N, dev), ridx_sample, ridx64)
    return ridx, pidx, samples, depths, deltas, boundary.view(torch.bool)


class MarchBuffers:

    def __init__(self, mode, N, per_ray, k, dev):
        self.mode, self.N, self.k = mode, int(N), int(k)
        ne = self.N * int(per_ray)
        self.cap = ne * self.k
        self.samples = torch.zeros(self.cap, 3, device=dev)
        self.depths = torch.zeros(self.cap, device=dev)
        self.deltas = torch.zeros(self.cap, device=dev)
        self.boundary = torch.zeros(self.cap, device=dev, dtype=torch.uint8)
        self.ridx_entry = torch.zeros(ne, device=dev, dtype=torch.int32)
        self.ridx_sample = self.ridx_entry if self.k == 1 else torch.zeros(self.cap, device=dev, dtype=torch.int32)
        self.ridx64 = torch.zeros(ne, device=dev, dtype=torch.int64)
        self.pidx = torch.zeros(ne, device=dev, dtype=torch.int32)
        self.counts = torch.zeros(self.N, device=dev, dtype=torch.int32)
        self.pack_start = torch.zeros(self.N + 1, device=dev, dtype=torch.int64)
        self.pack_start_c = torch.zeros(self.N + 1, device=dev, dtype=torch.int64)
        if mode == "voxel":
            self.nug_t = torch.empty(2, int(per_ray), self.N, 2, device=dev)
            self.nug_cell = torch.empty(2, int(per_ray), self.N, device=dev, dtype=torch.int32)

    def pad_to(self, capacity):
        assert 0 < capacity <= self.cap and capacity % self.k == 0
        _call("pag_pad_packed", L.ptr(self.pack_start), self.N, int(capacity), self.k, L.ptr(self.samples), L.ptr(self.depths), L.ptr(self.deltas),
              L.ptr(self.ridx_sample) if self.k > 1 else None, L.ptr(self.ridx_entry), L.ptr(self.ridx64), L.ptr(self.pidx), L.ptr(self.boundary),
              L.ptr(self.pack_start_c), L.stream())


def _offsets(buf, N, mb_ptr, st, pad_capacity, dirs, dirs_out):
    if pad_capacity is None:
        _call("pag_pack_offsets", L.ptr(buf.counts), N, L.ptr(buf.pack_start), mb_ptr, st)
        return
    assert 0 < pad_capacity <= buf.cap and pad_capacity % buf.k == 0
    copy = dirs_out is not None and dirs_out.data_ptr() != dirs.data_ptr()
    _call("pag_pack_offsets_pad", L.ptr(buf.counts), N, L.ptr(buf.pack_start), mb_ptr, int(pad_capacity), buf.k, L.ptr(buf.samples), L.ptr(buf.depths),
          L.ptr(buf.deltas), L.ptr(buf.ridx_sample) if buf.k > 1 else None, L.ptr(buf.ridx_entry), L.ptr(buf.ridx64), L.ptr(buf.pidx),
          L.ptr(buf.boundary), L.ptr(buf.pack_start_c), L.ptr(dirs) if copy else None, L.ptr(dirs_out) if copy else None, st)


def march_into(buf, origins, dirs, dist_min, dist_max, num_samples, jitter=None, occupancy_bits=None, blas_level=7, max_travel=None,
               occupancy_coarse_bits=None, pad_capacity=None, dirs_out=None):
    _check_gpu(origins, dirs)
    dev = origins.device
    N = origins.shape[0]
    assert N == buf.N
    origins = origins.detach().contiguous().float()
    dirs = dirs.detach().contiguous().float()
    occ = L.ptr(occupancy_bits) if occupancy_bits is not None else None
    st = L.stream()
    mailbox = _count_mailbox() if POLL_SAMPLE_COUNT else None
    if mailbox is not None:
        mailbox[1][0] = -1
    mb_ptr = mailbox[0].data_ptr() if mailbox is not None else None
    if buf.mode == "ray":
        S = int(num_samples)
        if jitter is None:
            jitter = torch.rand(N, S, device=dev)
        jitter = jitter.contiguous().float()
        tvals = _tvals(S, dev)
        _call("pag_raymarch_count", L.ptr(origins), L.ptr(dirs), N, S, L.ptr(tvals), L.ptr(jitter), float(dist_min), float(dist_max), occ,
              blas_level, L.ptr(buf.counts), st)
        _offsets(buf, N, mb_ptr, st, pad_capacity, dirs, dirs_out)
        _call("pag_raymarch_pack", L.ptr(origins), L.ptr(dirs), N, S, L.ptr(tvals), L.ptr(jitter), float(dist_min), float(dist_max), occ,
              blas_level, L.ptr(buf.pack_start), L.ptr(buf.ridx_entry), L.ptr(buf.pidx), L.ptr(buf.samples), L.ptr(buf.depths),
              L.ptr(buf.deltas), L.ptr(buf.boundary), L.ptr(buf.ridx64), st)
    else:
        k = buf.k
        coarse = L.ptr(occupancy_coarse_bits) if (occupancy_coarse_bits is not None and occupancy_bits is not None) else None
        travel = float("inf") if max_travel is None else float(max_travel)
        _call("pag_raymarch_voxel_count_nuggets", L.ptr(origins), L.ptr(dirs), N, k, float(dist_min), float(dist_max), occ, coarse,
              blas_level, travel, L.ptr(buf.counts), L.ptr(buf.nug_t), L.ptr(buf.nug_cell), st)
        _offsets(buf, N, mb_ptr, st, pad_capacity, dirs, dirs_out)
        _call("pag_raymarch_voxel_pack_nuggets", L.ptr(origins), L.ptr(dirs), N, k, L.ptr(buf.pack_start), L.ptr(buf.nug_t), L.ptr(buf.nug_cell), blas_level,
              L.ptr(buf.ridx_entry), L.ptr(buf.pidx), L.ptr(buf.samples), L.ptr(buf.depths), L.ptr(buf.deltas), L.ptr(buf.boundary),
              L.ptr(buf.ridx_sample), L.ptr(buf.ridx64), st)
    return mailbox, jitter


def copy_batch(dsts, srcs):
    easy, hard = [], []
    for d, s_ in zip(dsts, srcs):
        (easy if (d.dtype == s_.dtype and d.shape == s_.shape and d.is_contiguous() and s_.is_contiguous() and d.is_cuda and s_.is_cuda)
         else hard).append((d, s_))
    for c0 in range(0, len(easy), 16):
        part = easy[c0:c0 + 16]
        n = len(part)
        _call("pag_copy_batch", n, (ctypes.c_void_p * n)(*[d.data_ptr() for d, _ in part]), (ctypes.c_void_p * n)(*[s_.data_ptr() for _, s_ in part]),
              (ctypes.c_int64 * n)(*[d.numel() * d.element_size() for d, _ in part]), L.stream())
    for d, s_ in hard:
        d.copy_(s_)


def packs_from_boundary(ridx, boundary):
    starts = torch.nonzero(boundary).reshape(-1)
    end = torch.tensor([boundary.shape[0]], device=boundary.device, dtype=torch.int64)
    return torch.cat([starts, end]).contiguous(), ridx[starts].int().contiguous()


def occupancy_update(density, occupancy, bits, decay, min_density):
    _check_gpu(density, occupancy, bits)
    cells = occupancy.shape[0]
    density = density.detach()
    if density.dim() != 1 or density.dtype != torch.float32:
        density = density.reshape(cells, -1)[:, 0].float()
    assert occupancy.is_contiguous() and bits.is_contiguous() and bits.numel() * 32 >= cells
    _call("pag_occupancy_update", density.data_ptr(), density.stride(0), L.ptr(occupancy), L.ptr(bits), cells, float(decay),
          float(min_density), L.stream())


class _Composite(torch.autograd.Function):
    @staticmethod
    def forward(ctx, sigma, rgb, deltas, depths, pack_start, ray_of_pack, N, bg_white):
        _check_gpu(sigma, deltas)
        dev = sigma.device
        M = sigma.shape[0]
        P = ray_of_pack.shape[0]
        sigma = sigma.detach().contiguous().float()
        deltas = deltas.detach().contiguous().float()
        rgbc = rgb.detach().contiguous().float() if rgb is not None else None
        depc = depths.detach().contiguous().float() if depths is not None else None
        w = torch.empty(M, device=dev) if (P and M) else torch.zeros(M, device=dev)
        ctx.tail_zero = TAIL_ZERO
        if M and _one_pack_per_ray(ray_of_pack, N):
            alpha = torch.empty(N, device=dev)
            hit = torch.empty(N, device=dev, dtype=torch.uint8)
            out_rgb = torch.empty(N, 3, device=dev) if rgb is not None else None
            out_depth = torch.empty(N, device=dev) if depths is not None else None
        else:
            alpha = torch.zeros(N, device=dev)
            hit = torch.zeros(N, device=dev, dtype=torch.uint8)
            out_rgb = (torch.ones if bg_white else torch.zeros)(N, 3, device=dev) if rgb is not None else None
            out_depth = torch.zeros(N, device=dev) if depths is not None else None
        if P and M:
            _call("pag_composite_fwd", L.ptr(pack_start), L.ptr(ray_of_pack), P, L.ptr(sigma), L.ptr(deltas), L.ptr(depc),
                                          L.ptr(rgbc), L.BG_WHITE if bg_white else L.BG_BLACK, L.ptr(w), L.ptr(alpha),
                                          L.ptr(out_rgb), L.ptr(out_depth), L.ptr(hit), M if TAIL_ZERO else 0, L.stream())
        ctx.save_for_backward(sigma, rgbc, deltas, depc, pack_start, ray_of_pack, w, alpha)
        ctx.bg_white = bg_white
        ctx.mark_non_differentiable(hit, w)
        ctx.set_materialize_grads(False)
        return alpha, hit, out_rgb, out_depth, w

    @staticmethod
    def backward(ctx, g_alpha, _g_hit, g_rgb, g_depth, _g_w):
        sigma, rgbc, deltas, depc, pack_start, ray_of_pack, w, alpha = ctx.saved_tensors
        M, P = sigma.shape[0], ray_of_pack.shape[0]
        mk = torch.empty if (P and M) else torch.zeros
        d_sigma = mk(M, device=sigma.device)
        d_rgb = mk(M, 3, device=sigma.device) if rgbc is not None else None
        gc = lambda t: t.contiguous().float() if t is not None else None
        g_alpha, g_rgb, g_depth = gc(g_alpha), gc(g_rgb), gc(g_depth)
        if P and M:
            _call("pag_composite_bwd", L.ptr(pack_start), L.ptr(ray_of_pack), P, L.ptr(sigma), L.ptr(deltas), L.ptr(depc),
                                          L.ptr(rgbc), L.BG_WHITE if ctx.bg_white else L.BG_BLACK, L.ptr(w), L.ptr(alpha),
                                          L.ptr(g_rgb), L.ptr(g_depth), L.ptr(g_alpha), L.ptr(d_sigma), L.ptr(d_rgb),
                                          M if ctx.tail_zero else 0, L.stream())
        return d_sigma, d_rgb, None, None, None, None, None, None


def composite(sigma, rgb, deltas, depths, pack_start, ray_of_pack, N, bg_white=True):
    return _apply(_Composite, sigma, rgb, deltas, depths, pack_start, ray_of_pack, N, bg_white)


class _CompositeFeats(torch.autograd.Function):
    @staticmethod
    def forward(ctx, feats, weights, alpha, pack_start, ray_of_pack, N):
        _check_gpu(feats, weights, alpha)
        feats = feats.detach().contiguous()
        if feats.dtype not in (torch.float32, torch.bfloat16):
            feats = feats.float()
        C = feats.shape[1]
        P = ray_of_pack.shape[0]
        out = torch.zeros(N, C, device=feats.device)
        weights = weights.detach().contiguous()
        alpha = alpha.detach().contiguous()
        if P and feats.shape[0]:
            _call("pag_composite_feats_fwd", L.ptr(pack_start), L.ptr(ray_of_pack), P, L.ptr(weights), L.ptr(alpha),
                                                L.ptr(feats), L.dtype_code(feats), C, L.ptr(out), L.stream())
        ctx.save_for_backward(weights, alpha, pack_start, ray_of_pack)
        ctx.shape, ctx.fdtype = feats.shape, feats.dtype
        ctx.tail_zero = TAIL_ZERO
        return out

    @staticmethod
    def backward(ctx, g):
        weights, alpha, pack_start, ray_of_pack = ctx.saved_tensors
        M, C = ctx.shape
        P = ray_of_pack.shape[0]
        d = torch.empty(M, C, device=weights.device, dtype=ctx.fdtype) if (P and not ctx.tail_zero) else torch.zeros(M, C, device=weights.device, dtype=ctx.fdtype)
        if P and M:
            _call("pag_composite_feats_bwd", L.ptr(pack_start), L.ptr(ray_of_pack), P, L.ptr(weights), L.ptr(alpha),
                  L.ptr(g.contiguous().float()), C, L.ptr(d), L.dtype_code(d), L.stream())
        return d, None, None, None, None, None


def composite_feats(feats, weights, alpha, pack_start, ray_of_pack, N):
    return _apply(_CompositeFeats, feats, weights, alpha, pack_start, ray_of_pack, N)


class _CompositeFeatsWeights(torch.autograd.Function):

    @staticmethod
    def forward(ctx, sigma, deltas, feats, ridx, pack_start, ray_of_pack, N):
        _check_gpu(sigma, deltas, feats)
        dev = sigma.device
        M, P = sigma.shape[0], ray_of_pack.shape[0]
        sigma = sigma.detach().contiguous().float()
        deltas = deltas.detach().contiguous().float()
        feats = feats.detach().contiguous()
        if feats.dtype not in (torch.float32, torch.bfloat16):
            feats = feats.float()
        C = feats.shape[1]
        w = torch.empty(M, device=dev)
        alpha = torch.zeros(N, device=dev)
        hit = torch.zeros(N, device=dev, dtype=torch.uint8)
        out = torch.zeros(N, C, device=dev)
        if P and M:
            _call("pag_composite_fwd", L.ptr(pack_start), L.ptr(ray_of_pack), P, L.ptr(sigma), L.ptr(deltas), None, None, L.BG_BLACK,
                  L.ptr(w), L.ptr(alpha), None, None, L.ptr(hit), 0, L.stream())
            _call("pag_composite_feats_fwd", L.ptr(pack_start), L.ptr(ray_of_pack), P, L.ptr(w), L.ptr(alpha), L.ptr(feats),
                  L.dtype_code(feats), C, L.ptr(out), L.stream())
        ctx.save_for_backward(sigma, deltas, feats, ridx, pack_start, ray_of_pack, w, alpha)
        ctx.mark_non_differentiable(alpha)
        return out, alpha

    @staticmethod
    def backward(ctx, g, _g_alpha):
        sigma, deltas, feats, ridx, pack_start, ray_of_pack, w, alpha = ctx.saved_tensors
        M, C = feats.shape
        P = ray_of_pack.shape[0]
        dev = sigma.device
        g = g.contiguous().float()
        d_feats = torch.zeros(M, C, device=dev, dtype=feats.dtype)
        d_sigma = torch.zeros(M, device=dev)
        if P and M:
            if ctx.needs_input_grad[2]:
                _call("pag_composite_feats_bwd", L.ptr(pack_start), L.ptr(ray_of_pack), P, L.ptr(w), L.ptr(alpha), L.ptr(g), C,
                      L.ptr(d_feats), L.dtype_code(d_feats), L.stream())
            if ctx.needs_input_grad[0]:
                s3 = torch.zeros(M, 3, device=dev)
                rl = ridx.long()
                step = max(1, (1 << 24) // max(C, 1))
                for lo in range(0, M, step):
                    hi = min(M, lo + step)
                    s3[lo:hi, 0] = (feats[lo:hi].float() * g[rl[lo:hi]]).sum(1)
                ones = torch.zeros(alpha.shape[0], 3, device=dev)
                ones[:, 0] = 1.0
                d_rgb = torch.empty(M, 3, device=dev)
                _call("pag_composite_bwd", L.ptr(pack_start), L.ptr(ray_of_pack), P, L.ptr(sigma), L.ptr(deltas), None, L.ptr(s3),
                      L.BG_BLACK, L.ptr(w), L.ptr(alpha), L.ptr(ones), None, None, L.ptr(d_sigma), L.ptr(d_rgb), 0, L.stream())
        return d_sigma, None, (d_feats if ctx.needs_input_grad[2] else None), None, None, None, None


def composite_features(sigma, deltas, feats, ridx, pack_start, ray_of_pack, N):
    return _apply(_CompositeFeatsWeights, sigma, deltas, feats, ridx, pack_start, ray_of_pack, N)


HEAD_REBUILD = True
CD_FUSED = os.environ.get("PAG_CD_FUSED", "1") != "0"
_NEXT_HOLD = None
_NEXT_PRODUCER = None


def decoder_hold(x1):
    global _NEXT_HOLD
    _NEXT_HOLD = {"x1_ptr": x1.data_ptr()}
    return _NEXT_HOLD


def flush_hold(hold):
    global _NEXT_HOLD, _NEXT_PRODUCER
    if _NEXT_HOLD is hold:
        _NEXT_HOLD = None
    if hold is not None and _NEXT_PRODUCER is hold:
        _NEXT_PRODUCER = None
    if hold is not None and hold.get("args") is not None and not hold.get("taken"):
        _call("pag_mlp_fwd", ctypes.byref(hold["args"]), hold["M"], L.stream())
        hold["taken"] = True


HEAD_FWD_ONCE = os.environ.get("PAG_HEAD_FWD_ONCE", "1") != "0"
HEAD_FWD_ONCE_MIN_PER_RAY = int(os.environ.get("PAG_HEAD_FWD_ONCE_MIN_PER_RAY", "160"))
TAIL_ZERO = False
SAMPLES_HINT = None


class _HeadComposite(_FusedMLP):

    @staticmethod
    def forward(ctx, x1, weights_w, alpha, ridx, pack_start, ray_of_pack, N, in_dim, out_act, out_dtype, grouped, *wb):
        C = wb[len(wb) // 2 - 1].shape[0]
        M = x1.shape[1] if grouped is not None else x1.shape[0]
        P = ray_of_pack.shape[0]
        pre = None
        long_rays = (M if SAMPLES_HINT is None else SAMPLES_HINT) >= HEAD_FWD_ONCE_MIN_PER_RAY * P
        if HEAD_FWD_ONCE and long_rays and HEAD_REBUILD and C > 192 and P and M and out_act == L.ACT_SOFTMAX and out_dtype == torch.bfloat16:
            full = _one_pack_per_ray(ray_of_pack, N)
            pre = dict(pack_start=pack_start, ray_of_pack=ray_of_pack, weights=weights_w.detach().contiguous(), alpha=alpha.detach().contiguous(),
                       out=(torch.empty if full else torch.zeros)(N, C, device=x1.device))
            ctx.fwd_composite = pre
        probs = _HeadComposite._decode(ctx, x1, in_dim, out_act, out_dtype, grouped, *wb)
        ctx.fwd_composite = None
        if pre is not None and getattr(ctx, "composited", False):
            ctx.fwd_state = None
            ctx.hc = (pre["weights"], pre["alpha"], ridx)
            return pre["out"]
        return _HeadComposite._composite(ctx, probs, x1, weights_w, alpha, ridx, pack_start, ray_of_pack, N, grouped, *wb)

    @staticmethod
    def _decode(ctx, x1, in_dim, out_act, out_dtype, grouped, *wb):
        ctx.stats_only = HEAD_REBUILD
        ctx.rank1_expected = True
        return _FusedMLP.forward(ctx, x1, None, None, in_dim, out_act, L.MLP_MFMA_BF16, out_dtype, grouped, *wb)

    @staticmethod
    def _composite(ctx, probs, x1, weights_w, alpha, ridx, pack_start, ray_of_pack, N, grouped, *wb):
        C = wb[len(wb) // 2 - 1].shape[0]
        P = ray_of_pack.shape[0]
        M = x1.shape[1] if grouped is not None else x1.shape[0]
        full = M and _one_pack_per_ray(ray_of_pack, N) and (probs is None or C <= 16)
        out = (torch.empty if full else torch.zeros)(N, C, device=x1.device)
        weights_w = weights_w.detach().contiguous()
        alpha = alpha.detach().contiguous()
        if probs is None:
            hidden_last, W_last, b_last, stats = ctx.fwd_state
            ctx.fwd_state = None
            if P and M:
                _call("pag_head_composite_fwd", L.ptr(pack_start), L.ptr(ray_of_pack), P, L.ptr(hidden_last), L.ptr(W_last),
                      L.ptr(b_last), C, L.ptr(stats), L.ptr(weights_w), L.ptr(alpha), L.ptr(out),
                      int(M if SAMPLES_HINT is None else SAMPLES_HINT), L.stream())
        elif P and M:
            _call("pag_composite_feats_fwd", L.ptr(pack_start), L.ptr(ray_of_pack), P, L.ptr(weights_w), L.ptr(alpha),
                  L.ptr(probs), L.dtype_code(probs), C, L.ptr(out), L.stream())
        ctx.hc = (weights_w, alpha, ridx)
        return out

    @staticmethod
    def backward(ctx, g):
        dx1, gwb = _HeadComposite._backward_pair(ctx, g, None)
        return (dx1, None, None, None, None, None, None, None, None, None, None, *gwb)

    @staticmethod
    def _backward_pair(ctx, g, dx1_into, wgrad_queue=None, **kw):
        weights_w, alpha, ridx = ctx.hc
        grads = _FusedMLP._backward_impl(ctx, None, (g.contiguous().float(), weights_w.contiguous(), ridx.contiguous(), alpha.contiguous()),
                                         dx1_into, wgrad_queue=wgrad_queue, **kw)
        return grads[0], grads[8:]


class _SubCtx:

    def __init__(self, needs_x1, any_grad):
        self.needs_input_grad = (needs_x1, False)
        self.any_grad = any_grad
        self.saved_tensors = ()

    def save_for_backward(self, *tensors):
        self.saved_tensors = tensors


class _HeadCompositePair(torch.autograd.Function):

    @staticmethod
    def forward(ctx, x1, weights_w, alpha, ridx, pack_start, ray_of_pack, N, in_dims, out_dtype, grouped, n_a, *wb):
        any_grad = any(ctx.needs_input_grad)
        sub_a, sub_b = _SubCtx(ctx.needs_input_grad[0], any_grad), _SubCtx(ctx.needs_input_grad[0], any_grad)
        part_a, part_b = wb[:n_a], wb[n_a:]
        hold = {}
        sub_b.fwd_hold = hold
        probs_b = _HeadComposite._decode(sub_b, x1, in_dims[1], L.ACT_SOFTMAX, out_dtype, grouped, *part_b)
        sub_a.fwd_pair = hold
        out_a = _HeadComposite.forward(sub_a, x1, weights_w, alpha, ridx, pack_start, ray_of_pack, N, in_dims[0], L.ACT_SOFTMAX, out_dtype,
                                       grouped, *part_a)
        if hold.get("args") is not None and not hold.get("taken"):
            _call("pag_mlp_fwd", ctypes.byref(hold["args"]), hold["M"], L.stream())
        sub_a.fwd_pair = sub_b.fwd_hold = None
        out_b = _HeadComposite._composite(sub_b, probs_b, x1, weights_w, alpha, ridx, pack_start, ray_of_pack, N, grouped, *part_b)
        ctx.subs, ctx.n_a = [sub_a, sub_b], n_a
        return out_a, out_b

    @staticmethod
    def backward(ctx, g_a, g_b):
        sub_a, sub_b = ctx.subs
        queue = []
        x1 = sub_a.saved_tensors[0]
        dx = torch.empty(x1.shape, device=x1.device, dtype=x1.dtype) if sub_a.needs_input_grad[0] else None
        hold = {}
        gb = _HeadComposite._backward_pair(sub_b, g_b, dx, queue, hold=hold if dx is not None else None)
        ga = _HeadComposite._backward_pair(sub_a, g_a, None, queue, dx1_out=dx, pair_hold=hold)
        if hold.get("args") is not None and not hold.get("taken"):
            _call("pag_mlp_bwd", ctypes.byref(hold["args"]), hold["M"], L.stream())
        if queue:
            _launch_wgrad(queue, queue[0]["dz"].shape[0])
        return (ga[0], None, None, None, None, None, None, None, None, None, None, *ga[1], *gb[1])


def head_composite_pair(x1, heads, w, alpha, ridx, pack_start, ray_of_pack, N, out_dtype=torch.bfloat16, x1_grouped=None):
    (wa, ba, ia), (wb_, bb, ib) = heads
    return _apply_decoder(_HeadCompositePair, x1, w, alpha, ridx, pack_start, ray_of_pack, N, (int(ia), int(ib)), out_dtype, x1_grouped,
                                    len(wa) + len(ba), *wa, *ba, *wb_, *bb)


def head_composite(x1, weights, biases, w, alpha, ridx, pack_start, ray_of_pack, N, in_dim=None, out_act=L.ACT_NONE,
                   out_dtype=torch.bfloat16, x1_grouped=None):
    if in_dim is None:
        in_dim = weights[0].shape[1]
    return _apply_decoder(_HeadComposite, x1, w, alpha, ridx, pack_start, ray_of_pack, N, int(in_dim), out_act, out_dtype, x1_grouped,
                                *weights, *biases)


_LOSS_WS = {}

# ... 139 lines not shown
```

pagnerf_amd/tracer.py:

```python
import inspect

import torch
import torch.nn as nn

from . import ops
from .core import RenderBuffer


_TRACE_PARAMS = {}


class PanopticPackedRFTracer(nn.Module):
    def __init__(self, ray_sparcity_reg=0.0, ray_max_travel=6.0, raymarch_type="voxel", num_steps=64, step_size=1.0,
                 bg_color="white", use_graphs=None, graph_split=None, **kwargs):
        super().__init__()
        import os
        if use_graphs is None:
            use_graphs = os.environ.get("PAG_GRAPHS", "1")
            use_graphs = "static" if use_graphs == "static" else bool(int(use_graphs))
        self.use_graphs = "static" if use_graphs == "static" else bool(use_graphs)
        self.graph_split = graph_split
        self._graphs = None
        self.raymarch_type, self.num_steps, self.step_size, self.bg_color = raymarch_type, num_steps, step_size, bg_color
        self.render_channels = {"depth", "alpha", "hit"}
        self.base_channels = {"rgb", "density"}
        self.panoptic_channels = {"semantics", "inst_embedding"}
        self.ray_sparcity_reg = ray_sparcity_reg
        self.ray_max_travel = ray_max_travel

    def get_supported_channels(self):
        return {"depth", "hit", "rgb", "alpha", "semantics", "inst_embedding"}

    def get_required_nef_channels(self):
        return {"rgb", "density"}

    def forward(self, nef, channels=None, extra_channels=None, **kwargs):
        requested, extra, args = self._resolve(nef, channels, extra_channels, kwargs)
        return self.trace(nef, requested - extra, extra, **args)

    def _resolve(self, nef, channels, extra_channels, kwargs, skip=()):
        missing = self.get_required_nef_channels() - nef.get_supported_channels()
        if missing:
            raise Exception("nef does not supply the channels this tracer needs: %s" % missing)
        if channels is None:
            requested = self.get_supported_channels()
        elif isinstance(channels, str):
            requested = {channels}
        else:
            requested = set(channels)
        extra = requested - self.get_supported_channels()
        if extra_channels is not None:
            extra |= {extra_channels} if isinstance(extra_channels, str) else set(extra_channels)
        unsupported = extra - nef.get_supported_channels()
        if unsupported:
            raise Exception("channels %s are supported by neither the tracer nor the nef" % unsupported)
        args = {}
        sig = _TRACE_PARAMS.get(type(self))
        if sig is None:
            sig = _TRACE_PARAMS[type(self)] = tuple(inspect.signature(self.trace).parameters.items())
        for name, prm in sig:
            if name in ("nef", "channels", "extra_channels") or name in skip:
                continue
            if name in kwargs:
                args[name] = kwargs[name]
            elif hasattr(self, name):
                args[name] = getattr(self, name)
            elif prm.default is not inspect.Parameter.empty:
                args[name] = prm.default
        return requested, extra, args

    def trace(self, nef, channels, extra_channels, rays, lod_idx=None, raymarch_type="voxel", num_steps=64, step_size=1.0,
              bg_color="white", stage="val", jitter=None):
        assert nef.grid is not None, "this tracer requires a grid"
        N = rays.origins.shape[0]
        dev = rays.origins.device
        if lod_idx is None:
            lod_idx = nef.grid.num_lods - 1
        gkey = None
        if self.use_graphs and type(self).shade is PanopticPackedRFTracer.shade and raymarch_type in ("ray", "voxel"):
            from .graphs import GraphRunner
            if GraphRunner.eligible(self, nef, channels, extra_channels, rays, stage):
                if self._graphs is None:
                    self._graphs = GraphRunner()
                rb, gkey, jitter = self._graphs.run(self, nef, channels, rays, lod_idx, raymarch_type, num_steps, bg_color, stage, jitter)
                if rb is not None:
                    return rb
        marched = self._march(nef, rays, lod_idx, raymarch_type, num_steps, jitter)
        if gkey is not None:
            self._graphs.observe(gkey, marched[2].shape[0] * marched[6])
        return self._shade_marched(nef, channels, extra_channels, rays, marched, lod_idx, bg_color, stage)

    def _march(self, nef, rays, lod_idx, raymarch_type, num_steps, jitter=None, begun=None):
        dev = rays.origins.device
        kw = {"jitter": jitter} if jitter is not None else {}
        filtered = raymarch_type == "voxel" and getattr(nef.grid, "accepts_max_travel", False)
        if filtered:
            kw["max_travel"] = self.ray_max_travel
        if begun is not None:
            ridx, pidx, samples, depths, deltas, boundary = nef.grid.raymarch_voxel_finish(begun, rays, num_steps)
        else:
            ridx, pidx, samples, depths, deltas, boundary = nef.grid.raymarch(
                rays, level=nef.grid.active_lods[lod_idx], num_samples=num_steps, raymarch_type=raymarch_type, **kw)
        if samples.shape[0] and hasattr(nef, "prefetch_features") and (raymarch_type == "ray" or filtered) and self._prefetch:
            nef.prefetch_features(samples)
        if raymarch_type == "voxel" and depths.numel() != 0 and not filtered:
            _, counts_per_ray = ridx.unique(return_counts=True)
            ray_start_idx = torch.cumsum(counts_per_ray, dim=0)
            ray_start_idx = torch.cat([torch.zeros(1, dtype=ray_start_idx.dtype, device=dev), ray_start_idx[:-1]])
            hit_depth = torch.take(depths[:, 0, 0], ray_start_idx)
            traveled_depth = depths[:, 0, 0] - torch.repeat_interleave(hit_depth, counts_per_ray)
            valid_mask = traveled_depth < self.ray_max_travel
            deltas = deltas.reshape(depths.shape)[valid_mask].reshape(-1, 1)
            boundary = boundary.reshape(depths.shape)[valid_mask].reshape(-1)
            ridx, pidx, samples, depths = ridx[valid_mask], pidx[valid_mask], samples[valid_mask], depths[valid_mask]
        k = samples.shape[1] if samples.dim() == 3 else 1
        cache = getattr(nef.grid, "_pack_cache", None)
        if cache is not None and cache[0] is ridx:
            _, ridx32, pack_start, ray_of_pack = cache
        else:
            ridx32 = ridx.int() if k == 1 else ridx.int().repeat_interleave(k)
            pack_start, ray_of_pack = ops.packs_from_boundary(ridx32, boundary)
        return ridx, pidx, samples, depths, deltas, boundary, k, ridx32, pack_start, ray_of_pack

    def _shade_marched(self, nef, channels, extra_channels, rays, marched, lod_idx, bg_color, stage):
        ridx, pidx, samples, depths, deltas, _boundary, _k, ridx32, pack_start, ray_of_pack = marched
        outputs = self.shade(nef, channels, extra_channels, rays.dirs, rays.origins.shape[0], ridx, ridx32, pidx, samples, depths, deltas, pack_start,
                             ray_of_pack, lod_idx, bg_color, stage)
        return RenderBuffer(**outputs)

    _prefetch = True

    def render_packs(self, nef, packs, channels=None, extra_channels=None, **kwargs):
        packs = list(packs)
        if not packs:
            return []
        own = type(self).shade is PanopticPackedRFTracer.shade and type(self).trace is PanopticPackedRFTracer.trace
        if torch.is_grad_enabled() or not packs[0].origins.is_cuda or not own:
            return [self.forward(nef, channels=channels, extra_channels=extra_channels, rays=p, **kwargs) for p in packs]
        requested, extra, args = self._resolve(nef, channels, extra_channels, kwargs, skip=("rays",))
        lod_idx = args.get("lod_idx")
        if lod_idx is None:
            lod_idx = nef.grid.num_lods - 1
        rm, steps, bg, stage, jitter = args["raymarch_type"], args["num_steps"], args["bg_color"], args.get("stage", "val"), args.get("jitter")
        if jitter is not None:
            return [self.forward(nef, channels=channels, extra_channels=extra_channels, rays=p, **kwargs) for p in packs]
        dev = packs[0].origins.device
        main = torch.cuda.current_stream(dev)
        side = getattr(self, "_march_stream", None)
        if side is None or side.device != dev:
            side = self._march_stream = torch.cuda.Stream(device=dev, priority=-1)
        out = []

        side.wait_stream(main)

        split = rm == "voxel" and getattr(nef.grid, "accepts_max_travel", False) and hasattr(nef.grid, "raymarch_voxel_begin")
        if not split:
            return [self.forward(nef, channels=channels, extra_channels=extra_channels, rays=p, **kwargs) for p in packs]

        def begin(pack):
            if not split:
                return None
            with torch.cuda.stream(side):
                return nef.grid.raymarch_voxel_begin(pack, steps, self.ray_max_travel)

        def march(pack, begun):
            with torch.cuda.stream(side):
                m = self._march(nef, pack, lod_idx, rm, steps, None, begun=begun)
                ev = torch.cuda.Event()
                ev.record(side)
            for t in m:
                if isinstance(t, torch.Tensor):
                    t.record_stream(main)
            return m, ev
        self._prefetch = False
        try:
            b1 = begin(packs[1]) if len(packs) > 1 else None
            nxt = march(packs[0], begin(packs[0]))
            for i, pack in enumerate(packs):
                marched, ev = nxt
                main.wait_event(ev)
                out.append(self._shade_marched(nef, requested - extra, extra, pack, marched, lod_idx, bg, stage))
                if i + 1 < len(packs):
                    b2 = begin(packs[i + 2]) if i + 2 < len(packs) else None
                    nxt = march(packs[i + 1], b1)
                    b1 = b2
        finally:
            self._prefetch = True
        return out

    def shade(self, nef, channels, extra_channels, ray_dirs, N, ridx, ridx32, pidx, samples, depths, deltas, pack_start, ray_of_pack,
              lod_idx, bg_color, stage):
        dev = samples.device
        outputs = {}
        sample_channels = set(channels - self.render_channels)
        sample_channels.update(["density"])
        pan_req = [c for c in sorted(channels) if c in self.panoptic_channels]
        fuse_pan = bool(pan_req) and getattr(nef, "accepts_ray_index", False) and nef.can_fuse_panoptic(pan_req)
        if fuse_pan:
            sample_channels -= self.panoptic_channels
        if getattr(nef, "accepts_ray_index", False):
            feats = nef(coords=samples, ridx=ridx32, ray_dirs=ray_dirs, pidx=pidx, lod_idx=lod_idx, channels=sample_channels,
                        ray_packs=(pack_start, ray_of_pack))
        else:
            feats = nef(coords=samples, ray_d=ray_dirs.index_select(0, ridx), pidx=pidx, lod_idx=lod_idx,
                        channels=sample_channels)
        sigma = feats["density"].reshape(-1)
        if self.ray_sparcity_reg > 0.0 and stage == "train":
            per = torch.log(1.0 + 2 * sigma ** 2)
            ray_wise = torch.zeros(N, device=dev).scatter_add(0, ridx32.long(), per)
            outputs["ray_sparcity_loss"] = ray_wise.mean() * self.ray_sparcity_reg
        rgb = feats["rgb"].reshape(-1, 3) if "rgb" in channels else None
        dep = depths.reshape(-1) if "depth" in channels else None
        alpha, hit, out_rgb, out_depth, w = ops.composite(sigma, rgb, deltas.reshape(-1), dep, pack_start, ray_of_pack, N,
                                                          bg_white=(bg_color == "white"))
        outputs["alpha"] = alpha[:, None]
        outputs["hit"] = hit.view(torch.bool)
        if rgb is not None:
            outputs["rgb"] = out_rgb
        if dep is not None:
            outputs["depth"] = out_depth[:, None]
        alpha_d = alpha.detach()
        if fuse_pan:
            outputs.update(nef.panoptic_composited(samples, pan_req, w, alpha_d, ridx32, pack_start, ray_of_pack, N))
        else:
            for ch in pan_req:
                outputs[ch] = ops.composite_feats(feats[ch].reshape(-1, feats[ch].shape[-1]), w, alpha_d, pack_start, ray_of_pack, N)
        for ch in extra_channels:
            f = nef(coords=samples, ray_d=ray_dirs.index_select(0, ridx), pidx=pidx, lod_idx=lod_idx, channels=ch)
            outputs[ch] = ops.composite_features(sigma, deltas.reshape(-1), f.reshape(-1, f.shape[-1]), ridx32, pack_start,
                                                 ray_of_pack, N)[0]
        for attr in ("_feat_cache", "_density_feats"):
            if getattr(nef, attr, None) is not None:
                setattr(nef, attr, None)
        return outputs
```

Measured before the change: 1.223 million.

## Add live-sample stream compaction to skip dead samples in train shading

```diff
diff --git a/include/pagnerf_hip.h b/include/pagnerf_hip.h
--- a/include/pagnerf_hip.h
+++ b/include/pagnerf_hip.h
@@ -370,6 +370,16 @@
 int pag_sparse_rows_unpack(const float *buf, int L, int64_t T, int F, const uint32_t *bits, const int32_t *word_prefix, const int32_t *caps, const int64_t *offs,
                            float *grad, void *stream);
 
+int64_t pag_live_workspace_bytes(int64_t M);
+int pag_live_count(const void *pre, int pre_dtype, int64_t pre_stride, int64_t M, const int64_t *pack_start, int64_t N, void *workspace,
+                   int64_t workspace_bytes, int64_t *count_out, int64_t *count_host, void *stream);
+int pag_live_pack(const void *pre, int pre_dtype, int64_t pre_stride, int64_t M, const int64_t *pack_start, int64_t N, const void *workspace,
+                  int64_t capacity, int32_t *rank, int32_t *live_idx, int64_t *pack_start_live, void *stream);
+int pag_live_gather(int n, const void *const *src, void *const *dst, const int *words, const uint32_t *fill, const int32_t *live_idx,
+                    const void *workspace, int64_t M, int64_t capacity, void *stream);
+int pag_live_scatter(int n, const void *const *src, void *const *dst, const int *words, const int32_t *rank, int64_t M, int64_t capacity,
+                     void *stream);
+
 #ifdef __cplusplus
 }
 #endif
diff --git a/pagnerf_amd/_lib.py b/pagnerf_amd/_lib.py
--- a/pagnerf_amd/_lib.py
+++ b/pagnerf_amd/_lib.py
@@ -168,6 +168,11 @@
                                          c_vp, c_vp, c_i64, c_i32, c_vp]),
     "pag_permuto_encode_bwd_rays": (c_i32, [c_vp, c_i64, c_vp, c_i32, c_vp, c_i32, c_i64, c_i64, c_i32, c_i32, c_i32, c_u32, c_fp, c_fp, c_fp, c_vp, c_vp, c_vp,
                                             c_i64, c_vp, c_vp, c_i64, c_i32, c_vp]),
+    "pag_live_workspace_bytes": (c_i64, [c_i64]),
+    "pag_live_count": (c_i32, [c_vp, c_i32, c_i64, c_i64, c_vp, c_i64, c_vp, c_i64, c_vp, c_vp, c_vp]),
+    "pag_live_pack": (c_i32, [c_vp, c_i32, c_i64, c_i64, c_vp, c_i64, c_vp, c_i64, c_vp, c_vp, c_vp, c_vp]),
+    "pag_live_gather": (c_i32, [c_i32, c_vp, c_vp, c_vp, c_vp, c_vp, c_vp, c_i64, c_i64, c_vp]),
+    "pag_live_scatter": (c_i32, [c_i32, c_vp, c_vp, c_vp, c_vp, c_i64, c_i64, c_vp]),
 }
 
 EXPORTS = tuple(_SIGS)
diff --git a/pagnerf_amd/build.py b/pagnerf_amd/build.py
--- a/pagnerf_amd/build.py
+++ b/pagnerf_amd/build.py
@@ -29,6 +29,7 @@
     "panoptic.hip": ["-ffp-contract=off"],
     "map.hip": ["-ffp-contract=off"],
     "sparse.hip": [],
+    "compact.hip": [],
 }
 
 
diff --git a/pagnerf_amd/csrc/compact.hip b/pagnerf_amd/csrc/compact.hip
--- /dev/null
+++ b/pagnerf_amd/csrc/compact.hip
@@ -0,0 +1,235 @@
+#include "common.h"
+
+namespace {
+
+constexpr int TILE = 1024;
+constexpr int GATHER_MAX = 16;
+
+struct PreSrc {
+    const void *p;
+    int dtype;
+    int64_t stride;
+};
+
+__device__ __forceinline__ bool is_live(const PreSrc &s, int64_t m, int64_t M_real) {
+    if (m >= M_real) return false;
+    const float v = s.dtype == PAG_BF16 ? (float)reinterpret_cast<const bf16_t *>(s.p)[m * s.stride] : reinterpret_cast<const float *>(s.p)[m * s.stride];
+    return v > 0.0f;
+}
+
+__device__ __forceinline__ int64_t real_samples(const int64_t *pack_start, int64_t N, int64_t M) {
+    const int64_t t = pack_start ? pack_start[N] : M;
+    return t < M ? t : M;
+}
+
+__global__ __launch_bounds__(TILE) void live_count_kernel(PreSrc pre, int64_t M, const int64_t *__restrict__ pack_start, int64_t N, int32_t *__restrict__ tile_count) {
+    __shared__ int32_t wave_n[TILE / 64];
+    const int64_t m = (int64_t)blockIdx.x * TILE + threadIdx.x;
+    const bool live = is_live(pre, m, real_samples(pack_start, N, M));
+    const unsigned long long b = __ballot(live);
+    if ((threadIdx.x & 63) == 0) wave_n[threadIdx.x >> 6] = __popcll(b);
+    __syncthreads();
+    if (threadIdx.x == 0) {
+        int32_t s = 0;
+#pragma unroll
+        for (int w = 0; w < TILE / 64; ++w) s += wave_n[w];
+        tile_count[blockIdx.x] = s;
+    }
+}
+
+__global__ __launch_bounds__(1024) void live_scan_kernel(int32_t *__restrict__ tile, int64_t T, const int64_t *__restrict__ pack_start, int64_t N, int64_t M,
+                                                         int64_t *__restrict__ out, int64_t *mailbox) {
+    __shared__ int64_t part[1024];
+    const int tid = threadIdx.x;
+    const int64_t per = (T + 1023) / 1024, lo = tid * per, hi = lo + per < T ? lo + per : T;
+    int64_t s = 0;
+    for (int64_t t = lo; t < hi; ++t) s += tile[t];
+    part[tid] = s;
+    __syncthreads();
+    if (tid == 0) {
+        int64_t run = 0;
+        for (int i = 0; i < 1024; ++i) {
+            const int64_t c = part[i];
+            part[i] = run;
+            run += c;
+        }
+        tile[T] = (int32_t)run;
+        const int64_t real = real_samples(pack_start, N, M);
+        if (out) out[0] = run, out[1] = real;
+        if (mailbox) {
+            mailbox[1] = real;
+            __hip_atomic_store(mailbox, run, __ATOMIC_RELEASE, __HIP_MEMORY_SCOPE_SYSTEM);
+        }
+    }
+    __syncthreads();
+    int64_t run = part[tid];
+    for (int64_t t = lo; t < hi; ++t) {
+        const int32_t c = tile[t];
+        tile[t] = (int32_t)run;
+        run += c;
+    }
+}
+
+__global__ __launch_bounds__(TILE) void live_pack_kernel(PreSrc pre, int64_t M, const int64_t *__restrict__ pack_start, int64_t N, const int32_t *__restrict__ tile_off,
+                                                         int64_t capacity, int32_t *__restrict__ rank, int32_t *__restrict__ live_idx) {
+    __shared__ int32_t wave_n[TILE / 64];
+    const int64_t m = (int64_t)blockIdx.x * TILE + threadIdx.x;
+    const bool live = is_live(pre, m, real_samples(pack_start, N, M));
+    const unsigned long long b = __ballot(live);
+    const int lane = threadIdx.x & 63, wave = threadIdx.x >> 6;
+    if (lane == 0) wave_n[wave] = __popcll(b);
+    __syncthreads();
+    int32_t before = tile_off[blockIdx.x];
+    for (int w = 0; w < wave; ++w) before += wave_n[w];
+    before += __popcll(b & ((1ull << lane) - 1ull));
+    if (m < M) {
+        rank[m] = live ? before : ~before;
+        if (live && before < capacity) live_idx[before] = (int32_t)m;
+    }
+}
+
+__global__ __launch_bounds__(256) void live_table_kernel(const int64_t *__restrict__ pack_start, int64_t N, int64_t M, const int32_t *__restrict__ rank,
+                                                         const int32_t *__restrict__ tile_off, int64_t T, int64_t capacity, int64_t *__restrict__ pack_start_live) {
+    const int64_t r = (int64_t)blockIdx.x * 256 + threadIdx.x;
+    if (r > N) return;
+    const int64_t real = real_samples(pack_start, N, M), ps = pack_start[r];
+    int64_t v;
+    if (ps >= real) {
+        v = tile_off[T];
+    } else {
+        const int32_t k = rank[ps];
+        v = k >= 0 ? k : ~k;
+    }
+    pack_start_live[r] = v < capacity ? v : capacity;
+}
+
+struct RowBatch {
+    const void *src[GATHER_MAX];
+    void *dst[GATHER_MAX];
+    int words[GATHER_MAX];
+    uint32_t fill[GATHER_MAX];
+};
+
+__device__ __forceinline__ void copy_row(const uint32_t *s, uint32_t *d, int words) {
+    typedef unsigned int u32x4 __attribute__((ext_vector_type(4)));
+    if (words == 4 && ((reinterpret_cast<uintptr_t>(s) | reinterpret_cast<uintptr_t>(d)) & 15) == 0) {
+        *reinterpret_cast<u32x4 *>(d) = *reinterpret_cast<const u32x4 *>(s);
+        return;
+    }
+    for (int w = 0; w < words; ++w) d[w] = s[w];
+}
+
+__device__ __forceinline__ void fill_row(uint32_t *d, int words, uint32_t v) {
+    for (int w = 0; w < words; ++w) d[w] = v;
+}
+
+__global__ __launch_bounds__(256) void live_gather_kernel(RowBatch b, const int32_t *__restrict__ live_idx, const int32_t *__restrict__ tile_off, int64_t T,
+                                                          int64_t capacity, int64_t M) {
+    const int64_t i = (int64_t)blockIdx.x * 256 + threadIdx.x;
+    if (i >= capacity) return;
+    const int c = blockIdx.y, words = b.words[c];
+    uint32_t *d = reinterpret_cast<uint32_t *>(b.dst[c]) + i * words;
+    const int64_t count = tile_off[T];
+    if (i >= count) {
+        fill_row(d, words, b.fill[c]);
+        return;
+    }
+    const int64_t m = live_idx[i];
+    if (m < 0 || m >= M) {
+        fill_row(d, words, b.fill[c]);
+        return;
+    }
+    copy_row(reinterpret_cast<const uint32_t *>(b.src[c]) + m * words, d, words);
+}
+
+__global__ __launch_bounds__(256) void live_scatter_kernel(RowBatch b, const int32_t *__restrict__ rank, int64_t M, int64_t capacity) {
+    const int64_t m = (int64_t)blockIdx.x * 256 + threadIdx.x;
+    if (m >= M) return;
+    const int c = blockIdx.y, words = b.words[c];
+    uint32_t *d = reinterpret_cast<uint32_t *>(b.dst[c]) + m * words;
+    const int32_t k = rank[m];
+    if (k < 0 || k >= capacity) {
+        fill_row(d, words, 0u);
+        return;
+    }
+    copy_row(reinterpret_cast<const uint32_t *>(b.src[c]) + (int64_t)k * words, d, words);
+}
+
+inline int64_t tiles_of(int64_t M) { return (M + TILE - 1) / TILE; }
+
+int check_rows(const char *name, int n, const void *const *src, void *const *dst, const int *words, RowBatch &b, const uint32_t *fill) {
+    PAG_CHECK_ARG(n >= 1 && n <= GATHER_MAX, "%s: %d row tensors (1 .. %d per call)", name, n, GATHER_MAX);
+    PAG_CHECK_ARG(src && dst && words, "%s: NULL list", name);
+    for (int i = 0; i < n; ++i) {
+        PAG_CHECK_ARG(src[i] && dst[i], "%s: row tensor %d: NULL pointer", name, i);
+        PAG_CHECK_ARG(words[i] >= 1 && words[i] <= 4, "%s: row tensor %d: %d words per row (1 .. 4)", name, i, words[i]);
+        PAG_CHECK_ARG(((reinterpret_cast<uintptr_t>(src[i]) | reinterpret_cast<uintptr_t>(dst[i])) & 3) == 0, "%s: row tensor %d is not 4-byte aligned", name, i);
+        b.src[i] = src[i], b.dst[i] = dst[i], b.words[i] = words[i], b.fill[i] = fill ? fill[i] : 0u;
+    }
+    return PAG_OK;
+}
+
+}
+
+extern "C" int64_t pag_live_workspace_bytes(int64_t M) { return M < 0 ? -1 : (tiles_of(M) + 1) * (int64_t)sizeof(int32_t); }
+
+extern "C" int pag_live_count(const void *pre, int pre_dtype, int64_t pre_stride, int64_t M, const int64_t *pack_start, int64_t N, void *workspace,
+                              int64_t workspace_bytes, int64_t *count_out, int64_t *count_host, void *stream) {
+    PAG_CHECK_ARG(M >= 0 && M < (1ll << 31) && N >= 0 && pre_stride >= 1, "pag_live_count: M %lld, N %lld, stride %lld", (long long)M, (long long)N, (long long)pre_stride);
+    PAG_CHECK_ARG(pre_dtype == PAG_F32 || pre_dtype == PAG_BF16, "pag_live_count: pre must be f32 or bf16");
+    PAG_CHECK_ARG(workspace && workspace_bytes >= pag_live_workspace_bytes(M), "pag_live_count: workspace of %lld bytes, %lld needed", (long long)workspace_bytes,
+                  (long long)pag_live_workspace_bytes(M));
+    PAG_CHECK_ARG(M == 0 || pre, "pag_live_count: NULL pre");
+    const int64_t T = tiles_of(M);
+    PreSrc s{pre, pre_dtype, pre_stride};
+    int32_t *tile = reinterpret_cast<int32_t *>(workspace);
+    if (T) hipLaunchKernelGGL(live_count_kernel, dim3((unsigned)T), dim3(TILE), 0, (hipStream_t)stream, s, M, pack_start, N, tile);
+    hipLaunchKernelGGL(live_scan_kernel, dim3(1), dim3(1024), 0, (hipStream_t)stream, tile, T, pack_start, N, M, count_out, count_host);
+    PAG_CHECK_LAUNCH("pag_live_count");
+    return PAG_OK;
+}
+
+extern "C" int pag_live_pack(const void *pre, int pre_dtype, int64_t pre_stride, int64_t M, const int64_t *pack_start, int64_t N, const void *workspace,
+                             int64_t capacity, int32_t *rank, int32_t *live_idx, int64_t *pack_start_live, void *stream) {
+    PAG_CHECK_ARG(M >= 0 && M < (1ll << 31) && N >= 0 && pre_stride >= 1 && capacity >= 0, "pag_live_pack: M %lld, N %lld, stride %lld, capacity %lld", (long long)M,
+                  (long long)N, (long long)pre_stride, (long long)capacity);
+    PAG_CHECK_ARG(pre_dtype == PAG_F32 || pre_dtype == PAG_BF16, "pag_live_pack: pre must be f32 or bf16");
+    PAG_CHECK_ARG(workspace && pack_start && pack_start_live, "pag_live_pack: NULL workspace or pack table");
+    PAG_CHECK_ARG(M == 0 || (pre && rank), "pag_live_pack: NULL pre or rank");
+    PAG_CHECK_ARG(capacity == 0 || live_idx, "pag_live_pack: NULL live_idx");
+    const int64_t T = tiles_of(M);
+    PreSrc s{pre, pre_dtype, pre_stride};
+    const int32_t *tile = reinterpret_cast<const int32_t *>(workspace);
+    if (T) hipLaunchKernelGGL(live_pack_kernel, dim3((unsigned)T), dim3(TILE), 0, (hipStream_t)stream, s, M, pack_start, N, tile, capacity, rank, live_idx);
+    hipLaunchKernelGGL(live_table_kernel, dim3((unsigned)((N + 1 + 255) / 256)), dim3(256), 0, (hipStream_t)stream, pack_start, N, M, rank, tile, T, capacity,
+                       pack_start_live);
+    PAG_CHECK_LAUNCH("pag_live_pack");
+    return PAG_OK;
+}
+
+extern "C" int pag_live_gather(int n, const void *const *src, void *const *dst, const int *words, const uint32_t *fill, const int32_t *live_idx,
+                               const void *workspace, int64_t M, int64_t capacity, void *stream) {
+    RowBatch b{};
+    const int rc = check_rows("pag_live_gather", n, src, dst, words, b, fill);
+    if (rc != PAG_OK) return rc;
+    PAG_CHECK_ARG(M >= 0 && M < (1ll << 31) && capacity >= 0, "pag_live_gather: M %lld, capacity %lld", (long long)M, (long long)capacity);
+    if (capacity == 0) return PAG_OK;
+    PAG_CHECK_ARG(live_idx && workspace, "pag_live_gather: NULL live_idx or workspace");
+    hipLaunchKernelGGL(live_gather_kernel, dim3((unsigned)((capacity + 255) / 256), (unsigned)n), dim3(256), 0, (hipStream_t)stream, b, live_idx,
+                       reinterpret_cast<const int32_t *>(workspace), tiles_of(M), capacity, M);
+    PAG_CHECK_LAUNCH("pag_live_gather");
+    return PAG_OK;
+}
+
+extern "C" int pag_live_scatter(int n, const void *const *src, void *const *dst, const int *words, const int32_t *rank, int64_t M, int64_t capacity,
+                                void *stream) {
+    RowBatch b{};
+    const int rc = check_rows("pag_live_scatter", n, src, dst, words, b, nullptr);
+    if (rc != PAG_OK) return rc;
+    PAG_CHECK_ARG(M >= 0 && M < (1ll << 31) && capacity >= 0, "pag_live_scatter: M %lld, capacity %lld", (long long)M, (long long)capacity);
+    if (M == 0) return PAG_OK;
+    PAG_CHECK_ARG(rank, "pag_live_scatter: NULL rank");
+    hipLaunchKernelGGL(live_scatter_kernel, dim3((unsigned)((M + 255) / 256), (unsigned)n), dim3(256), 0, (hipStream_t)stream, b, rank, M, capacity);
+    PAG_CHECK_LAUNCH("pag_live_scatter");
+    return PAG_OK;
+}
diff --git a/pagnerf_amd/graphs.py b/pagnerf_amd/graphs.py
--- a/pagnerf_amd/graphs.py
+++ b/pagnerf_amd/graphs.py
@@ -13,20 +13,23 @@
 HISTORY = 8
 CAP_STEPS = 32
 SHRINK_WINDOW = 64
+LIVE_SHRINK_WINDOW = 256
 MAX_BUCKETS = 2
 
 
-def _round_capacity(want, k):
-    gran = GRANULE * k
-    step = max(gran, (1 << (max(int(want), 1).bit_length() - 1)) // CAP_STEPS // gran * gran)
+def _round_capacity(want, k, granule=GRANULE, cap_steps=CAP_STEPS):
+    gran = granule * k
+    step = max(gran, (1 << (max(int(want), 1).bit_length() - 1)) // cap_steps // gran * gran)
     return (int(want) + step - 1) // step * step
 
 
 class _PostMarch(nn.Module):
 
-    def __init__(self, nef, tracer, buf, capacity, channels, lod_idx, bg_color, stage):
+    def __init__(self, nef, tracer, buf, capacity, channels, lod_idx, bg_color, stage, live_cap=None, captured=False):
         super().__init__()
         self.nef = nef
+        self.live_cap, self.captured, self.probe_src = live_cap, captured, None
+        self.live_mailbox = ops.live_mailbox() if live_cap is not None else None
         self._t = (tracer, buf)
         self.capacity, self.channels, self.lod_idx, self.bg_color, self.stage = capacity, frozenset(channels), lod_idx, bg_color, stage
         self.names = None
@@ -39,8 +42,18 @@
         dep = depths.reshape(ne, k)
         if origins is not None:
             smp = ops.ray_samples(origins, ray_dirs, smp, dep, buf.pack_start_c, ops._ray_iota(N, samples.device), ridx=buf.ridx_sample[:cap])
-        out = tracer.shade(self.nef, set(self.channels), set(), ray_dirs, N, buf.ridx_entry[:ne], buf.ridx_sample[:cap], buf.pidx[:ne], smp, dep,
-                           deltas, buf.pack_start_c, ops._ray_iota(N, samples.device), self.lod_idx, self.bg_color, self.stage)
+        was = tracer._live_capture
+        if self.live_cap is not None:
+            from .tracer import LiveRequest
+            self.nef.live_compaction = LiveRequest(self.live_cap, self.live_mailbox)
+        tracer._live_capture = self if self.captured else None
+        try:
+            out = tracer.shade(self.nef, set(self.channels), set(), ray_dirs, N, buf.ridx_entry[:ne], buf.ridx_sample[:cap], buf.pidx[:ne], smp, dep,
+                               deltas, buf.pack_start_c, ops._ray_iota(N, samples.device), self.lod_idx, self.bg_color, self.stage)
+        finally:
+            tracer._live_capture = was
+            if self.live_cap is not None:
+                self.nef.live_compaction = None
         if self.names is None:
             self.names = sorted(out)
         return tuple(out[n] for n in self.names)
@@ -184,27 +197,29 @@
 
 
 class _State:
-    def __init__(self):
+    def __init__(self, shrink_window=SHRINK_WINDOW):
         self.counts = collections.deque(maxlen=HISTORY)
-        self.long = collections.deque(maxlen=SHRINK_WINDOW)
+        self.long = collections.deque(maxlen=shrink_window)
         self.cap = None
         self.buf = None
         self.dirs = None
         self.orig0 = None
         self.buckets = collections.OrderedDict()
+        self.live = None
 
     def see(self, count):
         self.counts.append(int(count))
         self.long.append(int(count))
 
     def capacity(self, buf):
-        want = _round_capacity(int(max(self.counts) * HEADROOM) + 1, buf.k)
+        gran, head, steps = getattr(buf, "granule", GRANULE), getattr(buf, "headroom", HEADROOM), getattr(buf, "cap_steps", CAP_STEPS)
+        want = _round_capacity(int(max(self.counts) * head) + 1, buf.k, gran, steps)
         if self.cap is None or want > self.cap:
             self.cap = want
             self.long.clear()
         elif len(self.long) == self.long.maxlen:
-            small = _round_capacity(int(max(self.long) * HEADROOM) + 1, buf.k)
-            if small < self.cap:
+            small = _round_capacity(int(max(self.long) * head) + 1, buf.k, gran, steps)
+            if small < self.cap * getattr(buf, "shrink_below", 1.0):
                 self.cap = small
                 self.long.clear()
         self.cap = min(buf.cap, self.cap)
@@ -221,6 +236,22 @@
             self.buckets.popitem(last=False)
         b = self.buckets[key] = make()
         return b
+
+
+class _LiveBuf:
+
+    """The live count moves with the MODEL, not only with the batch: while a scene trains it drifts by tens of per cent over a few hundred steps,
+    where the sample count of a fixed occupancy grid wobbles by a per cent or two.  Every new capacity is a capture (two warm-up steps, two
+    synchronisations: ~10 - 30 steps' worth of time), an overflow an eager step on top - so the live capacity keeps more head-room, coarser
+    buckets and a longer, stricter shrink rule than the sample capacity; fillers cost decoder time only (their gradient is zero: the
+    encoders' backward skips them)."""
+    granule = 256
+    headroom = 1.10
+    cap_steps = 8
+    shrink_below = 0.75
+
+    def __init__(self, cap):
+        self.k, self.cap = 1, cap
 
 
 class GraphRunner:
@@ -303,10 +334,19 @@
     def observe(self, key, count):
         self._state(key).see(count)
 
+    def observe_live(self, key, count):
+        st = self._state(key)
+        if st.live is None:
+            st.live = _State(shrink_window=LIVE_SHRINK_WINDOW)
+        st.live.see(count)
+
     def run(self, tracer, nef, channels, rays, lod_idx, raymarch_type, num_steps, bg_color, stage, jitter):
         key = self._key(tracer, nef, channels, rays, lod_idx, raymarch_type, num_steps, bg_color, stage)
         st = self._state(key)
         if not st.counts:
+            return None, key, jitter
+        live_on = tracer.use_graphs is True and tracer._live.enabled() and hasattr(nef, "_live_wanted") and "rgb" in channels
+        if live_on and (st.live is None or not st.live.counts):
             return None, key, jitter
         g = nef.grid
         dev = rays.origins.device
@@ -322,6 +362,8 @@
             st.orig0 = torch.zeros(N, 3, device=dev)
         buf = st.buf
         cap = st.capacity(buf)
+        lcap = min(cap, st.live.capacity(_LiveBuf(cap))) if live_on else None
+        bkey = cap if lcap is None else (cap, lcap)
         bits = None if g._all_occupied else g.blas_bits
         if bits is not None and bits.device != dev:
             g.blas_bits = bits = bits.to(dev)
@@ -346,7 +388,7 @@
                 self.overflows += 1
                 return None, key, jitter
             return RenderBuffer(**dict(zip(mod.names, outs))), key, jitter
-        graphed = st.bucket(cap)
+        graphed = st.bucket(bkey)
         if graphed is None:
             M = self._count(mailbox, buf)
             mailbox = None
@@ -363,15 +405,18 @@
                 st.buckets.popitem(last=False)
             gc.collect()
             torch.cuda.synchronize()
-            mod = _PostMarch(nef, tracer, buf, cap, channels, lod_idx, bg_color, stage)
+            mod = _PostMarch(nef, tracer, buf, cap, channels, lod_idx, bg_color, stage, live_cap=lcap, captured=True)
             mod.train(nef.training)
             ops.SAMPLES_HINT = M
             ops.TAIL_ZERO = True
             try:
-                graphed = st.bucket(cap, lambda: _Graphed(mod, args, split=self._split(tracer), grad_args=(3, 4) if pose else ()))
+                graphed = st.bucket(bkey, lambda: _Graphed(mod, args, split=self._split(tracer), grad_args=(3, 4) if pose else ()))
             finally:
                 ops.SAMPLES_HINT, ops.TAIL_ZERO = None, False
             self.captures += 1
+        lmb = graphed.mod.live_mailbox
+        if lmb is not None:
+            lmb[1][0] = -1
         outs = graphed(live)
         self.replays += 1
         if mailbox is not None:
@@ -380,6 +425,20 @@
             if M > cap:
                 self.overflows += 1
                 return None, key, jitter
+        src = graphed.mod.probe_src
+        if lmb is None and src is not None and tracer._live.probing():
+            ops.live_count(src[0], src[1], src[2], mailbox=tracer._live.mailbox)
+        if lmb is not None:
+            Ml = ops._poll_count(lmb, timeout_s=5.0)
+            if Ml < 0:
+                torch.cuda.current_stream().synchronize()
+                Ml = int(lmb[1][0])
+            st.live.see(Ml)
+            tracer._live.see(Ml, int(lmb[1][1]))
+            if Ml > graphed.mod.live_cap:
+                self.overflows += 1
+                self.live_overflows = getattr(self, "live_overflows", 0) + 1
+                return None, key, jitter
         return RenderBuffer(**dict(zip(graphed.mod.names, outs))), key, jitter
 
     @staticmethod
diff --git a/pagnerf_amd/nef.py b/pagnerf_amd/nef.py
--- a/pagnerf_amd/nef.py
+++ b/pagnerf_amd/nef.py
@@ -197,7 +197,55 @@
     def prefetch_features(self, coords):
         if self.multiscale_type != "cat" or self.grid is None:
             return
+        if self._live_wanted(coords):
+            with torch.no_grad():
+                self._prefetched = (coords, self._interp(self.grid, coords), False)
+            return
         self._prefetched = (coords, self._interp(self.grid, coords), torch.is_grad_enabled())
+
+    live_compaction = None
+
+    def _live_wanted(self, coords):
+        if self.live_compaction is None or not torch.is_grad_enabled() or not coords.is_cuda or coords.numel() == 0:
+            return False
+        if self.multiscale_type != "cat" or self._grouped() is None or self._heads_read_live_features():
+            return False
+        return (not coords.requires_grad) or hasattr(coords, "_pag_rays")
+
+    def _rgb_density_live(self, coords, feats, ridx, ray_dirs, ray_packs, mode):
+        req = self.live_compaction
+        grp = self._grouped()
+        pack_start, ray_of_pack = ray_packs
+        P = ray_of_pack.shape[0]
+        with torch.no_grad():
+            dens_full = self.decoder_density(feats, mode=mode, out_dtype=self.feat_dtype, x1_grouped=grp)
+        self._density_feats = dens_full
+        ls = ops.live_set(dens_full, pack_start, P, capacity=req.capacity, mailbox=req.mailbox)
+        req.result = ls
+        tag = getattr(coords, "_pag_rays", None) if coords.requires_grad else None
+        xyz = coords.detach().reshape(-1, 3).float()
+        last = max(int(ray_dirs.shape[0]) - 1, 0)
+        if tag is not None:
+            origins, dirs, depths = tag[0], tag[1], tag[2].detach().reshape(-1).float()
+            feats_c, xyz_c, ridx_c, dep_c = ops.live_gather(ls, [feats, xyz, ridx, depths], fills=[0, 0, last, 0])
+        else:
+            origins = dirs = dep_c = None
+            feats_c, xyz_c, ridx_c = ops.live_gather(ls, [feats, xyz, ridx], fills=[0, 0, last])
+        g = self.grid
+        flags = L.ENC_HALF_COORDS if g.rounds_coords() else 0
+        feats_c = ops.live_features(origins, dirs, feats_c, g.tables, g._spec, self._lod_weights_or_none(), flags, xyz_c, dep_c, ls.pack_start, ridx_c,
+                                    int(ray_dirs.shape[0]))
+        hold = ops.decoder_hold(feats_c) if ops.CD_FUSED else None
+        try:
+            density_feats = self.decoder_density(feats_c, mode=mode, out_dtype=self.feat_dtype, x1_grouped=grp)
+            pe, index = self._view_embedding(None, ridx_c, ray_dirs)
+            W, b = self.decoder_color.weights()
+            rgb_c, sigma_c = ops.colour_and_density(density_feats, W, b, pe, index, self.decoder_color.input_dim, out_act=L.ACT_SIGMOID, mode=mode,
+                                                    x2_packs=(ls.pack_start, ray_of_pack), producer=hold)
+        finally:
+            ops.flush_hold(hold)
+        sigma, rgb = ops.live_scatter_grad(sigma_c, rgb_c, ls)
+        return rgb, sigma
 
     def _panoptic_feats(self, feats_detached, coords):
         t = self.panoptic_features_type
@@ -224,12 +272,22 @@
         mode = self.mlp_mode
         pre = getattr(self, "_prefetched", None)
         self._prefetched = None
-        if pre is not None and pre[0] is coords and pre[2] == torch.is_grad_enabled():
-            feats = pre[1]
+        live = ("rgb" in compute_channels and ridx is not None and ray_dirs is not None and ray_packs is not None and ridx.dtype == torch.int32
+                and self._live_wanted(coords))
+        if pre is not None and pre[0] is coords and (pre[2] == (torch.is_grad_enabled() and not live) or live):
+            feats = pre[1].detach() if live else pre[1]
+        elif live:
+            with torch.no_grad():
+                feats = self._interp(self.grid, coords)
         else:
             feats = self._interp(self.grid, coords)
         self._feat_cache = (coords, feats if self._heads_read_live_features() else feats.detach())
         grp = self._grouped()
+        if live:
+            rgb, sigma = self._rgb_density_live(coords, feats, ridx, ray_dirs, ray_packs, mode)
+            out["rgb"] = rgb.reshape(batch, num_samples, 3)
+            density = sigma.reshape(batch, num_samples, 1)
+            return self._finish_channels(out, density, feats, coords, compute_channels, mode)
         hold = ops.decoder_hold(feats) if (ops.CD_FUSED and "rgb" in compute_channels and feats.is_cuda) else None
         try:
             density_feats = self.decoder_density(feats, mode=mode, out_dtype=self.feat_dtype, x1_grouped=grp)
@@ -247,6 +305,9 @@
                 density = torch.relu(density_feats[:, 0:1].float()).reshape(batch, num_samples, 1)
         finally:
             ops.flush_hold(hold)
+        return self._finish_channels(out, density, feats, coords, compute_channels, mode)
+
+    def _finish_channels(self, out, density, feats, coords, compute_channels, mode):
         if "density" in compute_channels:
             out["density"] = density
         if "semantics" in compute_channels or "inst_embedding" in compute_channels:
diff --git a/pagnerf_amd/ops.py b/pagnerf_amd/ops.py
--- a/pagnerf_amd/ops.py
+++ b/pagnerf_amd/ops.py
@@ -1203,6 +1203,165 @@
           float(min_density), L.stream())
 
 
+_LIVE_MAILBOX_FREE = []
+
+
+def live_mailbox():
+    t = torch.empty(2, dtype=torch.int64).pin_memory()
+    t[0], t[1] = -1, 0
+    return (t, t.numpy())
+
+
+def _pre_args(pre):
+    _check_gpu(pre)
+    pre = pre.detach()
+    if pre.dim() == 2:
+        assert pre.shape[1] == 1 or pre.stride(1) == 1
+    else:
+        assert pre.dim() == 1
+    M = pre.shape[0]
+    return pre.data_ptr() if M else None, _DTYPE_CODE[pre.dtype], max(int(pre.stride(0)), 1) if M else 1, M
+
+
+def live_count(pre, pack_start=None, P=0, mailbox=None):
+    p, dt, stride, M = _pre_args(pre)
+    nbytes = int(L.load().pag_live_workspace_bytes(M))
+    ws = torch.empty(nbytes // 4, dtype=torch.int32, device=pre.device)
+    _call("pag_live_count", p, dt, stride, M, L.ptr(pack_start), int(P) if pack_start is not None else 0, L.ptr(ws), nbytes, None,
+          mailbox[0].data_ptr() if mailbox is not None else None, L.stream())
+    return ws
+
+
+class LiveSet:
+    __slots__ = ("M", "P", "capacity", "rank", "live_idx", "pack_start", "ws", "count")
+
+
+def live_set(pre, pack_start, P, capacity=None, mailbox=None):
+    p, dt, stride, M = _pre_args(pre)
+    ls = LiveSet()
+    ls.M, ls.P, ls.count = M, int(P), None
+    own = mailbox is None
+    if own:
+        with _MAILBOX_LOCK:
+            mailbox = _LIVE_MAILBOX_FREE.pop() if _LIVE_MAILBOX_FREE else None
+        if mailbox is None:
+            mailbox = live_mailbox()
+    mailbox[1][0] = -1
+    ls.ws = live_count(pre, pack_start, P, mailbox)
+    if capacity is None:
+        v = _poll_count(mailbox, timeout_s=5.0)
+        if v < 0:
+            torch.cuda.current_stream().synchronize()
+            v = int(mailbox[1][0])
+        ls.count = capacity = v
+        if own:
+            with _MAILBOX_LOCK:
+                if len(_LIVE_MAILBOX_FREE) < 16:
+                    _LIVE_MAILBOX_FREE.append(mailbox)
+    ls.capacity = int(capacity)
+    dev = pre.device
+    ls.rank = torch.empty(M, dtype=torch.int32, device=dev)
+    ls.live_idx = torch.empty(ls.capacity, dtype=torch.int32, device=dev)
+    ls.pack_start = torch.empty(ls.P + 1, dtype=torch.int64, device=dev)
+    _call("pag_live_pack", p, dt, stride, M, L.ptr(pack_start), ls.P, L.ptr(ls.ws), ls.capacity, L.ptr(ls.rank) if M else None,
+          L.ptr(ls.live_idx) if ls.capacity else None, L.ptr(ls.pack_start), L.stream())
+    return ls
+
+
+def _row_lists(full, compact, M, cap):
+    out = []
+    for f, c in zip(full, compact):
+        assert f.is_contiguous() and c.is_contiguous() and f.dtype == c.dtype
+        if f.dim() == 3 and f.shape[0] == 8 and f.shape[2] == 8 and f.dtype == torch.bfloat16 and f.shape[1] == M:
+            out += [(f.data_ptr() + g * M * 16, c.data_ptr() + g * cap * 16, 4) for g in range(8)]
+        else:
+            assert f.shape[0] == M and c.shape[0] == cap
+            row = (f.numel() // M if M else c.numel() // max(cap, 1)) * f.element_size()
+            assert row % 4 == 0 and 4 <= row <= 16, "rows of 4 .. 16 bytes"
+            out.append((f.data_ptr(), c.data_ptr(), row // 4))
+    return out
+
+
+def _compact_like(t, M, cap):
+    if t.dim() == 3 and t.shape[0] == 8 and t.shape[2] == 8 and t.dtype == torch.bfloat16 and t.shape[1] == M:
+        return torch.empty(8, cap, 8, dtype=t.dtype, device=t.device)
+    return torch.empty((cap,) + tuple(t.shape[1:]), dtype=t.dtype, device=t.device)
+
+
+def live_gather(ls, tensors, fills=None):
+    tensors = [t.detach().contiguous() for t in tensors]
+    outs = [_compact_like(t, ls.M, ls.capacity) for t in tensors]
+    if ls.capacity == 0 or ls.M == 0:
+        return outs
+    rows, fl = [], []
+    for t, o, f in zip(tensors, outs, fills or [0] * len(tensors)):
+        r = _row_lists([t], [o], ls.M, ls.capacity)
+        rows += r
+        fl += [int(f) & 0xFFFFFFFF] * len(r)
+    for c0 in range(0, len(rows), 16):
+        part, n = rows[c0:c0 + 16], len(rows[c0:c0 + 16])
+        _call("pag_live_gather", n, (ctypes.c_void_p * n)(*[r[0] for r in part]), (ctypes.c_void_p * n)(*[r[1] for r in part]),
+              (ctypes.c_int * n)(*[r[2] for r in part]), (ctypes.c_uint32 * n)(*fl[c0:c0 + 16]), L.ptr(ls.live_idx), L.ptr(ls.ws), ls.M, ls.capacity,
+              L.stream())
+    return outs
+
+
+def live_scatter(ls, tensors):
+    tensors = [t.detach().contiguous() for t in tensors]
+    outs = [torch.empty((ls.M,) + tuple(t.shape[1:]), dtype=t.dtype, device=t.device) for t in tensors]
+    if ls.M == 0:
+        return outs
+    if ls.capacity == 0:
+        for o in outs:
+            o.zero_()
+        return outs
+    rows = _row_lists(outs, tensors, ls.M, ls.capacity)
+    n = len(rows)
+    _call("pag_live_scatter", n, (ctypes.c_void_p * n)(*[r[1] for r in rows]), (ctypes.c_void_p * n)(*[r[0] for r in rows]),
+          (ctypes.c_int * n)(*[r[2] for r in rows]), L.ptr(ls.rank), ls.M, ls.capacity, L.stream())
+    return outs
+
+
+class _LiveFeatures(torch.autograd.Function):
+
+    @staticmethod
+    def forward(ctx, origins, dirs, feats_c, tables, spec, feat_scale, flags, xyz_c, depths_c, pack_start, ridx_c, N):
+        ctx.spec, ctx.feat_scale, ctx.flags, ctx.N = spec, feat_scale, flags, N
+        ctx.save_for_backward(xyz_c, tables.detach().contiguous(), depths_c, pack_start, ridx_c)
+        ctx.tshape, ctx.tdtype = tables.shape, tables.dtype
+        return feats_c.view_as(feats_c)
+
+    @staticmethod
+    def backward(ctx, g):
+        r = _EncodeRays.backward(ctx, g)
+        return (r[0], r[1], None, r[3]) + (None,) * 8
+
+
+def live_features(origins, dirs, feats_c, tables, spec, feat_scale, flags, xyz_c, depths_c, pack_start, ridx_c, N):
+    return _LiveFeatures.apply(origins, dirs, feats_c, tables, spec, feat_scale, flags, xyz_c, depths_c, pack_start, ridx_c, N)
+
+
+class _LiveScatter(torch.autograd.Function):
+
+    @staticmethod
+    def forward(ctx, sigma_c, rgb_c, ls):
+        ctx.ls = ls
+        ctx.set_materialize_grads(False)
+        sigma, rgb = live_scatter(ls, [sigma_c.float(), rgb_c.float()])
+        return sigma, rgb
+
+    @staticmethod
+    def backward(ctx, g_sigma, g_rgb):
+        ls = ctx.ls
+        names = [g for g in (g_sigma, g_rgb) if g is not None]
+        got = iter(live_gather(ls, [g.float() for g in names])) if names else iter(())
+        return (next(got) if g_sigma is not None else None), (next(got) if g_rgb is not None else None), None
+
+
+def live_scatter_grad(sigma_c, rgb_c, ls):
+    return _LiveScatter.apply(sigma_c, rgb_c, ls)
+
+
 class _Composite(torch.autograd.Function):
     @staticmethod
     def forward(ctx, sigma, rgb, deltas, depths, pack_start, ray_of_pack, N, bg_white):
diff --git a/pagnerf_amd/tracer.py b/pagnerf_amd/tracer.py
--- a/pagnerf_amd/tracer.py
+++ b/pagnerf_amd/tracer.py
@@ -10,9 +10,71 @@
 _TRACE_PARAMS = {}
 
 
+class LiveRequest:
+    __slots__ = ("capacity", "mailbox", "result")
+
+    def __init__(self, capacity=None, mailbox=None):
+        self.capacity, self.mailbox, self.result = capacity, mailbox, None
+
+
+class LivePolicy:
+    WINDOW = 16
+    ON_BELOW = 0.65
+    OFF_ABOVE = 0.75
+    PROBE_EVERY = 8
+
+    def __init__(self, mode):
+        assert mode in ("auto", True, False), "live_compaction: 'auto', True or False"
+        self.mode = mode
+        self.active = mode is True
+        self.shares = []
+        self.mailbox = None
+        self.traces = 0
+        self.switches = 0
+
+    def enabled(self):
+        if self.mode is False:
+            return False
+        if torch.distributed.is_available() and torch.distributed.is_initialized() and torch.distributed.get_world_size() > 1:
+            return False
+        return self.active
+
+    def see(self, live, total):
+        if self.mode != "auto" or total <= 0:
+            return
+        share = float(live) / float(total)
+        if self.active:
+            if share > self.OFF_ABOVE:
+                self.active, self.shares = False, []
+                self.switches += 1
+            return
+        self.shares.append(share)
+        if share >= self.ON_BELOW:
+            self.shares = []
+        elif len(self.shares) >= self.WINDOW:
+            self.active, self.shares = True, []
+            self.switches += 1
+
+    def poll(self):
+        if self.mailbox is not None and int(self.mailbox[1][0]) >= 0:
+            live, total = int(self.mailbox[1][0]), int(self.mailbox[1][1])
+            self.mailbox[1][0] = -1
+            self.see(live, total)
+
+    def probing(self):
+        if self.mode != "auto" or self.active:
+            return False
+        self.traces += 1
+        if self.traces % self.PROBE_EVERY:
+            return False
+        if self.mailbox is None:
+            self.mailbox = ops.live_mailbox()
+        return True
+
+
 class PanopticPackedRFTracer(nn.Module):
     def __init__(self, ray_sparcity_reg=0.0, ray_max_travel=6.0, raymarch_type="voxel", num_steps=64, step_size=1.0,
-                 bg_color="white", use_graphs=None, graph_split=None, **kwargs):
+                 bg_color="white", use_graphs=None, graph_split=None, live_compaction="auto", **kwargs):
         super().__init__()
         import os
         if use_graphs is None:
@@ -21,6 +83,9 @@
         self.use_graphs = "static" if use_graphs == "static" else bool(use_graphs)
         self.graph_split = graph_split
         self._graphs = None
+        self.live_compaction = live_compaction
+        self._live = LivePolicy(live_compaction)
+        self._live_capture = None
         self.raymarch_type, self.num_steps, self.step_size, self.bg_color = raymarch_type, num_steps, step_size, bg_color
         self.render_channels = {"depth", "alpha", "hit"}
         self.base_channels = {"rgb", "density"}
@@ -76,6 +141,7 @@
         dev = rays.origins.device
         if lod_idx is None:
             lod_idx = nef.grid.num_lods - 1
+        self._live.poll()
         gkey = None
         if self.use_graphs and type(self).shade is PanopticPackedRFTracer.shade and raymarch_type in ("ray", "voxel"):
             from .graphs import GraphRunner
@@ -85,10 +151,23 @@
                 rb, gkey, jitter = self._graphs.run(self, nef, channels, rays, lod_idx, raymarch_type, num_steps, bg_color, stage, jitter)
                 if rb is not None:
                     return rb
-        marched = self._march(nef, rays, lod_idx, raymarch_type, num_steps, jitter)
-        if gkey is not None:
-            self._graphs.observe(gkey, marched[2].shape[0] * marched[6])
-        return self._shade_marched(nef, channels, extra_channels, rays, marched, lod_idx, bg_color, stage)
+        req = None
+        if (self._live.enabled() and self.use_graphs != "static" and stage == "train" and torch.is_grad_enabled() and not extra_channels
+                and type(self).shade is PanopticPackedRFTracer.shade and hasattr(nef, "_live_wanted")):
+            req = nef.live_compaction = LiveRequest()
+        try:
+            marched = self._march(nef, rays, lod_idx, raymarch_type, num_steps, jitter)
+            if gkey is not None:
+                self._graphs.observe(gkey, marched[2].shape[0] * marched[6])
+            rb = self._shade_marched(nef, channels, extra_channels, rays, marched, lod_idx, bg_color, stage)
+        finally:
+            if req is not None:
+                nef.live_compaction = None
+        if req is not None and req.result is not None:
+            self._live.see(req.result.count, req.result.M)
+            if gkey is not None:
+                self._graphs.observe_live(gkey, req.result.count)
+        return rb
 
     def _march(self, nef, rays, lod_idx, raymarch_type, num_steps, jitter=None, begun=None):
         dev = rays.origins.device
@@ -205,6 +284,11 @@
             feats = nef(coords=samples, ray_d=ray_dirs.index_select(0, ridx), pidx=pidx, lod_idx=lod_idx,
                         channels=sample_channels)
         sigma = feats["density"].reshape(-1)
+        if sigma.is_cuda and stage == "train" and torch.is_grad_enabled() and getattr(nef, "live_compaction", None) is None:
+            if self._live_capture is not None:
+                self._live_capture.probe_src = (sigma.detach(), pack_start, ray_of_pack.shape[0])
+            elif self._live.probing():
+                ops.live_count(sigma, pack_start, ray_of_pack.shape[0], mailbox=self._live.mailbox)
         if self.ray_sparcity_reg > 0.0 and stage == "train":
             per = torch.log(1.0 + 2 * sigma ** 2)
             ray_wise = torch.zeros(N, device=dev).scatter_add(0, ridx32.long(), per)
```

Result: slower. 1.206 million (-1.4%).
